# arnab39/Semi-supervised-segmentation-cycleGAN

Hardware: AMD Instinct MI355X
Metric: training images/sec (G+D step) at 256x256 (higher is better)
Workload: dtype f32; 1 GPU; VOC2012 21-class 256x256 semisupervised_cycleGAN as-written G+D step, batch=8 per GPU, fp32 tensors, 3-piece split-bf16 contraction, fp32-accurate (six exact bf16 piece products per fp32 product on the bf16 matrix cores, fp32 accumulation - forward, data and weight gradients; 21 / 20-channel stems and heads zero-padded onto the same contraction, 1- / 3-channel ends on the exact fp32 MFMA); global_batch=8, image_unit=one labeled + one unlabeled 256x256 image, parallelism=dp1, losses_finite=True

## Files before the change

### include/sscg.h

```cpp
#ifndef SSCG_H
#define SSCG_H
#include <stddef.h>
#include <stdint.h>

#ifdef __cplusplus
extern "C" {
#endif

#define SSCG_ABI_VERSION 18

#define SSCG_F32 0
#define SSCG_BF16 1
#define SSCG_BF16X3 2

#define SSCG_ERR_BAD_ARG (-1)
#define SSCG_ERR_UNSUPPORTED (-2)
#define SSCG_ERR_WORKSPACE (-3)

#define SSCG_ACT_NONE 0
#define SSCG_ACT_RELU 1
#define SSCG_ACT_LRELU 2
#define SSCG_ACT_TANH 3

#define SSCG_PAD_ZEROS 0
#define SSCG_PAD_REFLECT 1

int sscg_abi_version(void);
int sscg_set_dry_run(int on);

typedef struct sscg_conv_desc {
    int32_t N, H, W, C;
    int32_t K, R, S;
    int32_t P, Q;
    int32_t stride, pad, dil;
    int32_t pad_mode;
    int32_t act;
    float slope;
    int32_t x_dtype;
    int32_t w_dtype;
    int32_t y_dtype;
    int32_t precision;
    int32_t tuning;
    int64_t w_plane;
    int32_t wgrad_tuning;
} sscg_conv_desc;

size_t sscg_conv2d_fwd_workspace(const sscg_conv_desc* d);
int sscg_conv2d_fwd(const sscg_conv_desc* d, const void* x, const void* w, const float* bias, void* y, void* ws,
                    size_t ws_bytes, void* stream);

size_t sscg_conv2d_fwd_stats_bytes(const sscg_conv_desc* d, int G, int64_t L);
size_t sscg_conv2d_fwd_stats_workspace(const sscg_conv_desc* d);
int sscg_conv2d_fwd_stats(const sscg_conv_desc* d, const void* x, const void* w, const float* bias, void* y, int G, int64_t L,
                          void* stats, size_t stats_bytes, void* ws, size_t ws_bytes, void* stream);
int sscg_norm_stats_from_conv(const sscg_conv_desc* d, const void* stats, int G, int64_t L, float eps, float* mean, float* rstd,
                              float* running_mean, float* running_var, float momentum, void* stream);

int sscg_conv2d_fwd_affine_applies(const sscg_conv_desc* d);
int sscg_conv2d_fwd_affine(const sscg_conv_desc* d, const void* x, const void* w, const float* bias, const float* running_mean,
                           const float* running_var, float eps, const float* gamma, const float* beta, const void* residual, void* y,
                           void* ws, size_t ws_bytes, void* stream);

int sscg_conv2d_front_applies(const sscg_conv_desc* d, int cin);
int sscg_conv2d_front_fwd(const sscg_conv_desc* d, const void* xf, int cin, const float* w1, const float* b1, float slope1, void* h1,
                          const void* w, const float* bias, void* y, int G, int64_t L, void* stats, size_t stats_bytes, void* stream);

size_t sscg_conv2d_dgrad_workspace(const sscg_conv_desc* d);
int sscg_conv2d_dgrad(const sscg_conv_desc* d, const void* dy, const void* wt, const float* bias, void* dx,
                      int act, float slope, void* ws, size_t ws_bytes, void* stream);

size_t sscg_conv2d_wgrad_workspace(const sscg_conv_desc* d);
int sscg_conv2d_wgrad(const sscg_conv_desc* d, const void* x, const void* dy, float* dw, float beta, void* ws,
                      size_t ws_bytes, void* stream);

int sscg_weight_krsc_to_crsk(const void* w, int w_dtype, void* wt, int wt_dtype, int K, int RS, int C, void* stream);
typedef struct sscg_wt_job {
    const void* w;
    void* wt;
    int32_t w_dtype, wt_dtype;
    int32_t K, RS, C;
    int32_t block0;
} sscg_wt_job;
int sscg_weight_krsc_to_crsk_batch(const sscg_wt_job* jobs, int n_jobs, int n_blocks, void* stream);
int sscg_split3(const float* src, void* dst, int64_t n, int64_t plane_stride, void* stream);
int sscg_conv2d_split_applies(const sscg_conv_desc* d, int kind);
int sscg_cast(const void* src, int src_dtype, void* dst, int dst_dtype, int64_t n, void* stream);

size_t sscg_colsum_workspace(int64_t rows, int cols);
int sscg_colsum(const void* x, int dtype, float* out, int64_t rows, int cols, float beta, void* ws, size_t ws_bytes, void* stream);

size_t sscg_norm_stats_workspace(int G, int64_t L, int C);
int sscg_norm_stats(const void* x, int dtype, int G, int64_t L, int C, float eps, float* mean, float* rstd,
                    float* running_mean, float* running_var, float momentum, void* ws, size_t ws_bytes, void* stream);
int sscg_norm_apply(const void* x, const float* mean, const float* rstd, const float* gamma, const float* beta,
                    const void* residual, void* y, int dtype, int G, int64_t L, int C, int act, float slope, void* stream);
size_t sscg_conv2d_dgrad_bsums_bytes(const sscg_conv_desc* d, int G, int64_t L);
int sscg_conv2d_dgrad_bsums(const sscg_conv_desc* d, const void* dy, const void* wt, void* dx, const void* nx, const void* nz,
                            const void* addend, const float* mean, const float* rstd, const float* gamma, const float* beta, int G,
                            int64_t L, int act, float slope, void* sums, size_t sums_bytes, void* ws, size_t ws_bytes, void* stream);
int sscg_conv2d_dgrad_add_applies(const sscg_conv_desc* d);
int sscg_conv2d_dgrad_add(const sscg_conv_desc* d, const void* dy, const void* wt, const void* addend, void* dx, void* ws,
                          size_t ws_bytes, void* stream);
int sscg_norm_bwd_from_sums(const sscg_conv_desc* d, const void* sums, const void* dy, const void* x, const void* y, const float* mean,
                            const float* rstd, const float* gamma, const float* beta, void* dx, void* dres, float* dgamma, float* dbeta,
                            int dtype, int G, int64_t L, int C, int act, float slope, int flags, void* ws, size_t ws_bytes, void* stream);

int sscg_rstd_from_var(const float* var, float* rstd, int n, float eps, void* stream);
size_t sscg_norm_bwd_workspace(int G, int64_t L, int C);
int sscg_norm_bwd(const void* dy, const void* x, const void* y, const float* mean, const float* rstd,
                  const float* gamma, const float* beta, void* dx, void* dres, float* dgamma, float* dbeta, int dtype, int G,
                  int64_t L, int C, int act, float slope, int stats_grad, void* ws, size_t ws_bytes, void* stream);

int sscg_norm_head_applies(int C);
int sscg_norm_head_fwd(const void* x, int dtype, const float* mean, const float* rstd, const float* gamma, const float* beta,
                       const float* w, const float* bias, float* out, int G, int64_t L, int C, int act, float slope, void* stream);
size_t sscg_norm_head_bwd_workspace(int G, int64_t L, int C);
int sscg_norm_head_bwd(const float* dout, const float* w, const void* x, const float* mean, const float* rstd, const float* gamma,
                       const float* beta, void* dx, float* dw, float* dbias, float* dgamma, float* dbeta, int dtype, int G, int64_t L,
                       int C, int act, float slope, int flags, void* ws, size_t ws_bytes, void* stream);

int sscg_act_fwd(const void* x, void* y, int dtype, int64_t n, int act, float slope, void* stream);
int sscg_act_bwd(const void* dy, const void* y, void* dx, int dtype, int64_t n, int act, float slope, void* stream);
int sscg_add(const void* a, const void* b, void* y, int dtype, int64_t n, void* stream);
int sscg_resize_channels(const float* src, float* dst, int64_t rows, int Cs, int Cd, void* stream);
int sscg_dropout(const void* x, void* y, int dtype, int64_t n, float p, uint64_t seed, void* stream);
int sscg_gauss_noise(const float* x, float* y, int64_t n, float sigma, uint64_t seed, void* stream);
int sscg_maxpool2x2_fwd(const void* x, void* y, uint8_t* idx, int dtype, int N, int H, int W, int C, void* stream);
int sscg_maxpool2x2_bwd(const void* dy, const uint8_t* idx, void* dx, int dtype, int N, int H, int W, int C, void* stream);
int sscg_maxpool3x3s2_fwd(const void* x, void* y, uint8_t* idx, int dtype, int N, int H, int W, int C, int P, int Q, void* stream);
int sscg_maxpool3x3s2_bwd(const void* dy, const uint8_t* idx, void* dx, int dtype, int N, int H, int W, int C, int P, int Q, void* stream);
int sscg_upsample_bilinear_fwd(const float* x, float* y, int N, int H, int W, int C, int OH, int OW, void* stream);
int sscg_upsample_bilinear_bwd(const float* dy, float* dx, int N, int H, int W, int C, int OH, int OW, void* stream);
int sscg_reflect_pad(const void* x, void* y, int dtype, int N, int H, int W, int C, int pad, void* stream);
int sscg_reflect_pad_bwd(const void* dy, void* dx, int dtype, int N, int H, int W, int C, int pad, void* stream);
int sscg_nchw_to_nhwc(const float* x, float* y, int N, int C, int H, int W, void* stream);
int sscg_nhwc_to_nchw(const float* x, float* y, int N, int C, int H, int W, void* stream);

int sscg_softmax_fwd(const float* x, float* y, int64_t rows, int C, void* stream);
int sscg_softmax_bwd(const float* dy, const float* y, float* dx, int64_t rows, int C, void* stream);
int sscg_argmax_onehot(const float* x, float* onehot, int64_t* index, int64_t rows, int C, void* stream);
int sscg_label_onehot(const int64_t* labels, float* onehot, int64_t rows, int C, void* stream);
int sscg_confusion_hist(const int64_t* label_true, const int64_t* label_pred, int64_t n, int C, int64_t* hist, void* stream);

int sscg_image_u8_to_f32(const uint8_t* src, float* dst, int64_t rows, int C, const float* mean, const float* stdev, void* stream);
int sscg_label_lut(const uint8_t* src, int64_t* dst, int64_t n, const int64_t* lut256, void* stream);

size_t sscg_loss_workspace(int64_t n);
int sscg_ce_fwd(const float* logits, const int64_t* labels, int64_t rows, int C, float* loss, float* valid, void* ws,
                size_t ws_bytes, void* stream);
int sscg_ce_bwd(const float* logits, const int64_t* labels, int64_t rows, int C, const float* gscale, float w,
                const float* valid, float* dx, void* stream);
size_t sscg_upsample_head_workspace(int N, int H, int W);
int sscg_upsample_head_fwd(const float* x, const int64_t* labels, float* y_soft, float* loss, float* valid, float* dlogits, int N, int H,
                           int W, int C, int OH, int OW, void* ws, size_t ws_bytes, void* stream);
int sscg_upsample_head_bwd(const float* x, const float* dy_soft, const float* dlogits, const float* g_ce, const float* valid, float* dx,
                           int N, int H, int W, int C, int OH, int OW, void* stream);
int sscg_predict_head(const float* x, int N, int H, int W, int C, int OH, int OW, int64_t* index, uint8_t* label_u8,
                      const int64_t* label_true, int64_t* hist, void* stream);
int sscg_image_head(const float* x, int N, int H, int W, int C, int OH, int OW, float* y_nhwc, uint8_t* rgb_u8, void* stream);
int sscg_mse_const_fwd(const float* x, int64_t n, float target, float* loss, void* ws, size_t ws_bytes, void* stream);
int sscg_mse_const_bwd(const float* x, int64_t n, float target, const float* gscale, float w, float* dx, void* stream);
int sscg_mse_fwd(const float* a, const float* b, int64_t n, float* loss, void* ws, size_t ws_bytes, void* stream);
int sscg_mse_bwd(const float* a, const float* b, int64_t n, const float* gscale, float w, float* da, float* db, void* stream);
int sscg_l1_fwd(const float* a, const float* b, int64_t n, float* loss, void* ws, size_t ws_bytes, void* stream);
int sscg_l1_bwd(const float* a, const float* b, int64_t n, const float* gscale, float w, float* da, void* stream);
int sscg_weighted_sum(const float* const* terms, const float* w, int n, float* out, void* stream);

int sscg_adam_step(float* param, const float* grad, float* exp_avg, float* exp_avg_sq, void* shadow, int shadow_dtype, int64_t n,
                   double lr, double beta1, double beta2, double eps, int step, float grad_scale, void* stream);
int sscg_fill(float* x, int64_t n, float v, void* stream);

#ifdef __cplusplus
}
#endif
#endif
```

### semi-supervised-segmentation-cyclegan_amd/_lib.py

```python
import ctypes as C
import os

_HERE = os.path.dirname(os.path.abspath(__file__))
LIB_PATH = os.environ.get("SSCG_LIB") or os.path.join(_HERE, "libsscg.so")

ABI_VERSION = 18

F32, BF16, BF16X3 = 0, 1, 2

ACT_NONE, ACT_RELU, ACT_LRELU, ACT_TANH = 0, 1, 2, 3
PAD_ZEROS, PAD_REFLECT = 0, 1


class ConvDesc(C.Structure):

    _fields_ = [
        ("N", C.c_int32), ("H", C.c_int32), ("W", C.c_int32), ("C", C.c_int32),
        ("K", C.c_int32), ("R", C.c_int32), ("S", C.c_int32),
        ("P", C.c_int32), ("Q", C.c_int32),
        ("stride", C.c_int32), ("pad", C.c_int32), ("dil", C.c_int32),
        ("pad_mode", C.c_int32), ("act", C.c_int32), ("slope", C.c_float),
        ("x_dtype", C.c_int32), ("w_dtype", C.c_int32), ("y_dtype", C.c_int32), ("precision", C.c_int32),
        ("tuning", C.c_int32), ("w_plane", C.c_int64), ("wgrad_tuning", C.c_int32),
    ]


_p = C.c_void_p
_i = C.c_int
_i64 = C.c_int64
_f = C.c_float
_sz = C.c_size_t
_dp = C.POINTER(ConvDesc)

SIGNATURES = {
    "sscg_abi_version": (_i, []),
    "sscg_set_dry_run": (_i, [_i]),
    "sscg_resize_channels": (_i, [_p, _p, _i64, _i, _i, _p]),
    "sscg_conv2d_fwd_workspace": (_sz, [_dp]),
    "sscg_conv2d_fwd": (_i, [_dp, _p, _p, _p, _p, _p, _sz, _p]),
    "sscg_conv2d_fwd_stats_bytes": (_sz, [_dp, _i, _i64]),
    "sscg_conv2d_fwd_stats_workspace": (_sz, [_dp]),
    "sscg_conv2d_fwd_stats": (_i, [_dp, _p, _p, _p, _p, _i, _i64, _p, _sz, _p, _sz, _p]),
    "sscg_norm_stats_from_conv": (_i, [_dp, _p, _i, _i64, _f, _p, _p, _p, _p, _f, _p]),
    "sscg_conv2d_fwd_affine_applies": (_i, [_dp]),
    "sscg_conv2d_fwd_affine": (_i, [_dp, _p, _p, _p, _p, _p, _f, _p, _p, _p, _p, _p, _sz, _p]),
    "sscg_conv2d_front_applies": (_i, [_dp, _i]),
    "sscg_conv2d_front_fwd": (_i, [_dp, _p, _i, _p, _p, _f, _p, _p, _p, _p, _i, _i64, _p, _sz, _p]),
    "sscg_conv2d_dgrad_workspace": (_sz, [_dp]),
    "sscg_conv2d_dgrad": (_i, [_dp, _p, _p, _p, _p, _i, _f, _p, _sz, _p]),
    "sscg_conv2d_dgrad_bsums_bytes": (_sz, [_dp, _i, _i64]),
    "sscg_conv2d_dgrad_bsums": (_i, [_dp, _p, _p, _p, _p, _p, _p, _p, _p, _p, _p, _i, _i64, _i, _f, _p, _sz, _p, _sz, _p]),
    "sscg_conv2d_dgrad_add_applies": (_i, [_dp]),
    "sscg_conv2d_dgrad_add": (_i, [_dp, _p, _p, _p, _p, _p, _sz, _p]),
    "sscg_norm_bwd_from_sums": (_i, [_dp, _p, _p, _p, _p, _p, _p, _p, _p, _p, _p, _p, _p, _i, _i, _i64, _i, _i, _f, _i, _p, _sz, _p]),
    "sscg_conv2d_wgrad_workspace": (_sz, [_dp]),
    "sscg_conv2d_wgrad": (_i, [_dp, _p, _p, _p, _f, _p, _sz, _p]),
    "sscg_weight_krsc_to_crsk": (_i, [_p, _i, _p, _i, _i, _i, _i, _p]),
    "sscg_weight_krsc_to_crsk_batch": (_i, [_p, _i, _i, _p]),
    "sscg_split3": (_i, [_p, _p, _i64, _i64, _p]),
    "sscg_conv2d_split_applies": (_i, [_dp, _i]),
    "sscg_cast": (_i, [_p, _i, _p, _i, _i64, _p]),
    "sscg_colsum_workspace": (_sz, [_i64, _i]),
    "sscg_colsum": (_i, [_p, _i, _p, _i64, _i, _f, _p, _sz, _p]),
    "sscg_norm_stats_workspace": (_sz, [_i, _i64, _i]),
    "sscg_norm_stats": (_i, [_p, _i, _i, _i64, _i, _f, _p, _p, _p, _p, _f, _p, _sz, _p]),
    "sscg_norm_apply": (_i, [_p, _p, _p, _p, _p, _p, _p, _i, _i, _i64, _i, _i, _f, _p]),
    "sscg_rstd_from_var": (_i, [_p, _p, _i, _f, _p]),
    "sscg_norm_bwd_workspace": (_sz, [_i, _i64, _i]),
    "sscg_norm_bwd": (_i, [_p, _p, _p, _p, _p, _p, _p, _p, _p, _p, _p, _i, _i, _i64, _i, _i, _f, _i, _p, _sz, _p]),
    "sscg_norm_head_applies": (_i, [_i]),
    "sscg_norm_head_fwd": (_i, [_p, _i, _p, _p, _p, _p, _p, _p, _p, _i, _i64, _i, _i, _f, _p]),
    "sscg_norm_head_bwd_workspace": (_sz, [_i, _i64, _i]),
    "sscg_norm_head_bwd": (_i, [_p, _p, _p, _p, _p, _p, _p, _p, _p, _p, _p, _p, _i, _i, _i64, _i, _i, _f, _i, _p, _sz, _p]),
    "sscg_act_fwd": (_i, [_p, _p, _i, _i64, _i, _f, _p]),
    "sscg_act_bwd": (_i, [_p, _p, _p, _i, _i64, _i, _f, _p]),
    "sscg_add": (_i, [_p, _p, _p, _i, _i64, _p]),
    "sscg_dropout": (_i, [_p, _p, _i, _i64, _f, C.c_uint64, _p]),
    "sscg_gauss_noise": (_i, [_p, _p, _i64, _f, C.c_uint64, _p]),
    "sscg_maxpool2x2_fwd": (_i, [_p, _p, _p, _i, _i, _i, _i, _i, _p]),
    "sscg_maxpool2x2_bwd": (_i, [_p, _p, _p, _i, _i, _i, _i, _i, _p]),
    "sscg_maxpool3x3s2_fwd": (_i, [_p, _p, _p, _i, _i, _i, _i, _i, _i, _i, _p]),
    "sscg_maxpool3x3s2_bwd": (_i, [_p, _p, _p, _i, _i, _i, _i, _i, _i, _i, _p]),
    "sscg_upsample_bilinear_fwd": (_i, [_p, _p, _i, _i, _i, _i, _i, _i, _p]),
    "sscg_upsample_bilinear_bwd": (_i, [_p, _p, _i, _i, _i, _i, _i, _i, _p]),
    "sscg_reflect_pad": (_i, [_p, _p, _i, _i, _i, _i, _i, _i, _p]),
    "sscg_reflect_pad_bwd": (_i, [_p, _p, _i, _i, _i, _i, _i, _i, _p]),
    "sscg_nchw_to_nhwc": (_i, [_p, _p, _i, _i, _i, _i, _p]),
    "sscg_nhwc_to_nchw": (_i, [_p, _p, _i, _i, _i, _i, _p]),
    "sscg_softmax_fwd": (_i, [_p, _p, _i64, _i, _p]),
    "sscg_softmax_bwd": (_i, [_p, _p, _p, _i64, _i, _p]),
    "sscg_argmax_onehot": (_i, [_p, _p, _p, _i64, _i, _p]),
    "sscg_label_onehot": (_i, [_p, _p, _i64, _i, _p]),
    "sscg_confusion_hist": (_i, [_p, _p, _i64, _i, _p, _p]),
    "sscg_image_u8_to_f32": (_i, [_p, _p, _i64, _i, _p, _p, _p]),
    "sscg_label_lut": (_i, [_p, _p, _i64, _p, _p]),
    "sscg_loss_workspace": (_sz, [_i64]),
    "sscg_ce_fwd": (_i, [_p, _p, _i64, _i, _p, _p, _p, _sz, _p]),
    "sscg_ce_bwd": (_i, [_p, _p, _i64, _i, _p, _f, _p, _p, _p]),
    "sscg_upsample_head_workspace": (_sz, [_i, _i, _i]),
    "sscg_upsample_head_fwd": (_i, [_p, _p, _p, _p, _p, _p, _i, _i, _i, _i, _i, _i, _p, _sz, _p]),
    "sscg_upsample_head_bwd": (_i, [_p, _p, _p, _p, _p, _p, _i, _i, _i, _i, _i, _i, _p]),
    "sscg_predict_head": (_i, [_p, _i, _i, _i, _i, _i, _i, _p, _p, _p, _p, _p]),
    "sscg_image_head": (_i, [_p, _i, _i, _i, _i, _i, _i, _p, _p, _p]),
    "sscg_mse_const_fwd": (_i, [_p, _i64, _f, _p, _p, _sz, _p]),
    "sscg_mse_const_bwd": (_i, [_p, _i64, _f, _p, _f, _p, _p]),
    "sscg_mse_fwd": (_i, [_p, _p, _i64, _p, _p, _sz, _p]),
    "sscg_mse_bwd": (_i, [_p, _p, _i64, _p, _f, _p, _p, _p]),
    "sscg_l1_fwd": (_i, [_p, _p, _i64, _p, _p, _sz, _p]),
    "sscg_l1_bwd": (_i, [_p, _p, _i64, _p, _f, _p, _p]),
    "sscg_weighted_sum": (_i, [C.POINTER(_p), C.POINTER(_f), _i, _p, _p]),
    "sscg_adam_step": (_i, [_p, _p, _p, _p, _p, _i, _i64, C.c_double, C.c_double, C.c_double, C.c_double, _i, _f, _p]),
    "sscg_fill": (_i, [_p, _i64, _f, _p]),
}


class SscgError(RuntimeError):
    pass


def _load():
    if not os.path.exists(LIB_PATH):
        raise ImportError(
            "libsscg.so not found at %s - build it with `make -C %s/csrc` or "
            "`python -c 'import __graft_entry__ as g; g.build()'`. There is no fallback path." % (LIB_PATH, _HERE))
    lib = C.CDLL(LIB_PATH)
    for name, (res, args) in SIGNATURES.items():
        fn = getattr(lib, name)
        fn.restype = res
        fn.argtypes = args
    v = lib.sscg_abi_version()
    if v != ABI_VERSION:
        raise ImportError("libsscg.so ABI version %d != binding version %d" % (v, ABI_VERSION))
    if os.environ.get("SSCG_TRACE"):
        return _Traced(lib)
    if os.environ.get("SSCG_RACECHECK"):
        racecheck = dev_tool("racecheck")
        racecheck.install()
        return racecheck._Checked(lib)
    if os.environ.get("SSCG_FUZZ"):
        return dev_tool("racecheck")._Fuzzed(lib)
    return lib


def dev_tool(name):
    import importlib.util
    import sys
    if name in sys.modules:
        return sys.modules[name]
    path = os.path.join(os.path.dirname(_HERE), "tools", name + ".py")
    spec = importlib.util.spec_from_file_location(name, path)
    if spec is None or not os.path.exists(path):
        raise ImportError("development tool %s not found at %s" % (name, path))
    mod = importlib.util.module_from_spec(spec)
    sys.modules[name] = mod
    spec.loader.exec_module(mod)
    return mod


class _Traced:

    def __init__(self, lib):
        self._lib = lib

    def __getattr__(self, name):
        fn = getattr(self._lib, name)

        def call(*a):
            import sys
            import torch
            sys.stderr.write("[sscg] %s%s\n" % (name, tuple(x if isinstance(x, (int, float)) else "." for x in a)))
            sys.stderr.flush()
            r = fn(*a)
            if torch.cuda.is_available():
                torch.cuda.synchronize()
            return r
        return call


lib = _load()

_ERRS = {-1: "SSCG_ERR_BAD_ARG", -2: "SSCG_ERR_UNSUPPORTED", -3: "SSCG_ERR_WORKSPACE"}


def check(rc, what):
    if rc != 0:
        raise SscgError("%s failed: %s" % (what, _ERRS.get(rc, "hipError_t %d" % rc)))
```

### semi-supervised-segmentation-cyclegan_amd/csrc/common.h

```cpp
#pragma once
#include <hip/hip_runtime.h>
#include <stdint.h>
#include <stddef.h>

extern int g_sscg_dry_run;
#undef hipLaunchKernelGGL
#define hipLaunchKernelGGL(kernelName, numBlocks, numThreads, memPerBlock, streamId, ...)                                   \
    do {                                                                                                                     \
        if (!g_sscg_dry_run) { (kernelName)<<<(numBlocks), (numThreads), (memPerBlock), (streamId)>>>(__VA_ARGS__); }        \
    } while (0)

typedef float f32x16 __attribute__((ext_vector_type(16)));
typedef __bf16 bf16x8 __attribute__((ext_vector_type(8)));

struct sscg_bf3 { __bf16 h, m, l; };
__device__ __forceinline__ sscg_bf3 sscg_split3(float x) {
    sscg_bf3 t;
    t.h = (__bf16)x;
    const float r1 = x - (float)t.h;
    t.m = (__bf16)r1;
    const float r2 = r1 - (float)t.m;
    t.l = (__bf16)r2;
    return t;
}
typedef float f32x4 __attribute__((ext_vector_type(4)));
typedef __bf16 bf16x4 __attribute__((ext_vector_type(4)));

typedef uint32_t sscg_u32x4 __attribute__((ext_vector_type(4)));
__device__ __forceinline__ uint32_t sscg_cvt_pk_bf16(float a, float b) {
    typedef __bf16 bf16x2_t __attribute__((ext_vector_type(2)));
    typedef float f32x2_t __attribute__((ext_vector_type(2)));
    const f32x2_t v = {a, b};
    return __builtin_bit_cast(uint32_t, __builtin_convertvector(v, bf16x2_t));
}
__device__ __forceinline__ void sscg_split8(const float (&x)[8], bf16x8& h, bf16x8& m, bf16x8& l) {
    sscg_u32x4 ph, pm, pl;
#pragma unroll
    for (int w = 0; w < 4; ++w) {
        const float a = x[2 * w], b = x[2 * w + 1];
        const uint32_t hh = sscg_cvt_pk_bf16(a, b);
        const float ra = a - __builtin_bit_cast(float, hh << 16), rb = b - __builtin_bit_cast(float, hh & 0xffff0000u);
        const uint32_t mm = sscg_cvt_pk_bf16(ra, rb);
        const float sa = ra - __builtin_bit_cast(float, mm << 16), sb = rb - __builtin_bit_cast(float, mm & 0xffff0000u);
        ph[w] = hh; pm[w] = mm; pl[w] = sscg_cvt_pk_bf16(sa, sb);
    }
    h = __builtin_bit_cast(bf16x8, ph);
    m = __builtin_bit_cast(bf16x8, pm);
    l = __builtin_bit_cast(bf16x8, pl);
}

template <typename T> __device__ __forceinline__ float ld1(const T* p);
template <> __device__ __forceinline__ float ld1<float>(const float* p) { return *p; }
template <> __device__ __forceinline__ float ld1<__bf16>(const __bf16* p) { return (float)*p; }
template <typename T> __device__ __forceinline__ void st1(T* p, float v);
template <> __device__ __forceinline__ void st1<float>(float* p, float v) { *p = v; }
template <> __device__ __forceinline__ void st1<__bf16>(__bf16* p, float v) { *p = (__bf16)v; }
template <typename T> __device__ __forceinline__ void ld4(const T* p, float v[4]);
template <> __device__ __forceinline__ void ld4<float>(const float* p, float v[4]) {
    const f32x4 t = *reinterpret_cast<const f32x4*>(p);
    v[0] = t[0]; v[1] = t[1]; v[2] = t[2]; v[3] = t[3];
}
template <> __device__ __forceinline__ void ld4<__bf16>(const __bf16* p, float v[4]) {
    const bf16x4 t = *reinterpret_cast<const bf16x4*>(p);
    v[0] = (float)t[0]; v[1] = (float)t[1]; v[2] = (float)t[2]; v[3] = (float)t[3];
}
template <typename T> __device__ __forceinline__ void st4(T* p, const float v[4]);
template <> __device__ __forceinline__ void st4<float>(float* p, const float v[4]) {
    const f32x4 t = {v[0], v[1], v[2], v[3]};
    *reinterpret_cast<f32x4*>(p) = t;
}
template <> __device__ __forceinline__ void st4<__bf16>(__bf16* p, const float v[4]) {
    const bf16x4 t = {(__bf16)v[0], (__bf16)v[1], (__bf16)v[2], (__bf16)v[3]};
    *reinterpret_cast<bf16x4*>(p) = t;
}
typedef __bf16 bf16x8_t __attribute__((ext_vector_type(8)));
template <typename T> __device__ __forceinline__ void ld8(const T* p, float v[8]);
template <> __device__ __forceinline__ void ld8<float>(const float* p, float v[8]) { ld4<float>(p, v); ld4<float>(p + 4, v + 4); }
template <> __device__ __forceinline__ void ld8<__bf16>(const __bf16* p, float v[8]) {
    const bf16x8_t t = *reinterpret_cast<const bf16x8_t*>(p);
#pragma unroll
    for (int e = 0; e < 8; ++e) v[e] = (float)t[e];
}
template <typename T> __device__ __forceinline__ void st8(T* p, const float v[8]);
template <> __device__ __forceinline__ void st8<float>(float* p, const float v[8]) { st4<float>(p, v); st4<float>(p + 4, v + 4); }
template <> __device__ __forceinline__ void st8<__bf16>(__bf16* p, const float v[8]) {
    bf16x8_t t;
#pragma unroll
    for (int e = 0; e < 8; ++e) t[e] = (__bf16)v[e];
    *reinterpret_cast<bf16x8_t*>(p) = t;
}

#define SSCG_OK 0
#define SSCG_ERR_BAD_ARG (-1)
#define SSCG_ERR_UNSUPPORTED (-2)
#define SSCG_ERR_WORKSPACE (-3)

#define SSCG_LAUNCH_CHECK()                        \
    do {                                           \
        hipError_t e__ = hipGetLastError();        \
        if (e__ != hipSuccess) return (int)e__;    \
    } while (0)

enum { SSCG_ACT_NONE = 0, SSCG_ACT_RELU = 1, SSCG_ACT_LRELU = 2, SSCG_ACT_TANH = 3 };

__device__ __forceinline__ float sscg_act(float v, int act, float slope) {
    if (act == SSCG_ACT_RELU) return v > 0.f ? v : 0.f;
    if (act == SSCG_ACT_LRELU) return v > 0.f ? v : v * slope;
    if (act == SSCG_ACT_TANH) return tanhf(v);
    return v;
}

struct FastDiv {
    uint32_t mul;
    uint32_t shift;
    int32_t d;
};

static inline FastDiv make_fastdiv(int d) {
    FastDiv f;
    f.d = d;
    uint32_t l = 0;
    while ((1u << l) < (uint32_t)d) ++l;
    f.shift = l;
    f.mul = (uint32_t)((((uint64_t)1 << 32) * (((uint64_t)1 << l) - (uint64_t)d)) / (uint64_t)d + 1);
    return f;
}

__device__ __forceinline__ int fd_div(int n, const FastDiv& f) {
    return (int)((__umulhi((uint32_t)n, f.mul) + (uint32_t)n) >> f.shift);
}

__device__ __forceinline__ int xcd_remap(int bid, int nwg) {
    const int q = nwg >> 3, r = nwg & 7;
    const int xcd = bid & 7, idx = bid >> 3;
    return (xcd < r ? xcd * (q + 1) : r * (q + 1) + (xcd - r) * q) + idx;
}

static inline int cdiv(long a, long b) { return (int)((a + b - 1) / b); }

__device__ __forceinline__ double wave_sum(double v) {
#pragma unroll
    for (int o = 32; o > 0; o >>= 1) v += __shfl_xor(v, o, 64);
    return v;
}
__device__ __forceinline__ float wave_sum(float v) {
#pragma unroll
    for (int o = 32; o > 0; o >>= 1) v += __shfl_xor(v, o, 64);
    return v;
}

#define SSCG_ENSURE_SMEM(kern, smem)                                                                                                   \
    do {                                                                                                                               \
        static size_t sscg_attr_smem_[16] = {0};                                                                                       \
        int sscg_dev_ = 0;                                                                                                             \
        if (hipGetDevice(&sscg_dev_) != hipSuccess) sscg_dev_ = 0;                                                                     \
        size_t& sscg_cur_ = sscg_attr_smem_[sscg_dev_ & 15];                                                                           \
        if (sscg_cur_ == 0) sscg_cur_ = 64 * 1024;                                                                                     \
        if ((size_t)(smem) > sscg_cur_) {                                                                                              \
            hipError_t sscg_e_ = hipFuncSetAttribute(reinterpret_cast<const void*>(kern), hipFuncAttributeMaxDynamicSharedMemorySize, \
                                                     (int)(smem));                                                                     \
            if (sscg_e_ != hipSuccess) return (int)sscg_e_;                                                                            \
            sscg_cur_ = (size_t)(smem);                                                                                                \
        }                                                                                                                              \
    } while (0)

template <int BM, int BN, int NT, int TM, int TN>
__device__ __forceinline__ void sscg_stage_store_tile(const f32x16 (&acc)[TM][TN], float* ot, float* __restrict__ out, int m0, int n0, int Mlim,
                                                      int Ng, int row_w, int col_w, int li, int lh, int tid, float beta) {
    constexpr int OLD = BN + 4;
    __syncthreads();
#pragma unroll
    for (int j = 0; j < TN; ++j)
#pragma unroll
        for (int i = 0; i < TM; ++i)
#pragma unroll
            for (int e = 0; e < 16; ++e)
                ot[(row_w + i * 32 + (e & 3) + 8 * (e >> 2) + 4 * lh) * OLD + col_w + j * 32 + li] = acc[i][j][e];
    __syncthreads();
    constexpr int TPR = BN / 4;
    constexpr int RPP = NT / TPR;
    const int c4 = (tid % TPR) * 4;
    const int n = n0 + c4;
    if (n >= Ng) return;
#pragma unroll
    for (int ps = 0; ps < BM / RPP; ++ps) {
        const int r = tid / TPR + ps * RPP;
        const int m = m0 + r;
        if (m >= Mlim) break;
        f32x4 v = *reinterpret_cast<const f32x4*>(ot + r * OLD + c4);
        float* o = out + (size_t)m * Ng + n;
        if (beta != 0.f) v += beta * *reinterpret_cast<const f32x4*>(o);
        *reinterpret_cast<f32x4*>(o) = v;
    }
}
```

### semi-supervised-segmentation-cyclegan_amd/csrc/conv_split.hip

```cpp
#include "common.h"
#include "sscg_internal.h"
#include "reduce_common.h"
#include "bn_fold.h"
#include <cstdlib>
#include <type_traits>

namespace {

#ifndef KS_ABLATE
#define KS_ABLATE 0
#endif
#ifndef KS_BUFLD
#define KS_BUFLD 1
#endif
#ifndef KS_ACC2
#define KS_ACC2 1
#endif
#ifndef KS_LATE_WAIT
#define KS_LATE_WAIT 0
#endif
#ifndef KS_LB4
#define KS_LB4 1
#endif
constexpr int BKS = 32;
// ... 1754 lines not shown
#pragma unroll
            for (int pl = 0; pl < 3; ++pl) {
                asm volatile("ds_read_b64_tr_b16 %0, %1 offset:%2" : "=v"(fb[j][pl][0]) : "v"(lds0 + b_off[j]), "n"(pl * WS_PLANE));
                asm volatile("ds_read_b64_tr_b16 %0, %1 offset:%2" : "=v"(fb[j][pl][1]) : "v"(lds0 + b_off[j]), "n"(pl * WS_PLANE + 4 * WS_ROWB));
            }
        if (next) read_raw((it + 1) % WF_NRAW);
        __builtin_amdgcn_sched_barrier(0);
        wait_lgkm<0>();
        bf16x8 va[TM][3], vb[TN][3];
#pragma unroll
        for (int i = 0; i < TM; ++i)
#pragma unroll
            for (int pl = 0; pl < 3; ++pl) {
                va[i][pl] = __builtin_shufflevector(fa[i][pl][0], fa[i][pl][1], 0, 1, 2, 3, 4, 5, 6, 7);
                pin(va[i][pl]);
            }
#pragma unroll
        for (int j = 0; j < TN; ++j)
#pragma unroll
            for (int pl = 0; pl < 3; ++pl) {
                vb[j][pl] = __builtin_shufflevector(fb[j][pl][0], fb[j][pl][1], 0, 1, 2, 3, 4, 5, 6, 7);
                pin(vb[j][pl]);
            }
        if (next) { pin(raw[0][0]); pin(raw[0][1]); pin(raw[1][0]); pin(raw[1][1]); }
        __builtin_amdgcn_sched_barrier(0);
#pragma unroll
        for (int t = 0; t < 6; ++t) {
            const int ap = t == 0 ? 2 : (t == 1 || t == 3) ? 1 : 0;
            const int bp = (t == 0 || t == 3 || t == 5) ? 0 : (t == 1 || t == 4) ? 1 : 2;
#pragma unroll
            for (int i = 0; i < TM; ++i)
#pragma unroll
                for (int j = 0; j < TN; ++j)
                    acc[i][j] = __builtin_amdgcn_mfma_f32_32x32x16_bf16(va[i][ap], vb[j][bp], acc[i][j], 0, 0, 0);
            if (t == 0) {
                __builtin_amdgcn_sched_barrier(0);
                if (next) split_raw();
            }
        }
        if (next) {
#pragma unroll
            for (int n = 0; n < 20; ++n) {
                __builtin_amdgcn_sched_group_barrier(0x008, 1, 0);
                __builtin_amdgcn_sched_group_barrier(0x002, 5, 0);
            }
#pragma unroll
            for (int op = 0; op < 2; ++op)
#pragma unroll
                for (int pl = 0; pl < 3; ++pl) pin(pc[op][pl]);
        }
        __builtin_amdgcn_sched_barrier(0);
        if (!next) break;
        __builtin_amdgcn_s_barrier();
        if (issued < nsteps) { request_tile(); ++issued; }
        write_pieces();
        wait_lgkm<0>();
        if (it + 2 < nsteps) wait_tile(it + 2);
        __builtin_amdgcn_s_barrier();
    }

    float* out = p.out + (size_t)split * p.Kc * p.C;
    const bool direct = (p.splits == 1);
    ws_store_tile(acc, reinterpret_cast<float*>(smem_raw), out, m0, n0, p.Kc, p.C, row_w, col_w, li, lh, tid, direct ? p.beta : 0.f);
}

struct WgsPlan { int splits, chunk; };

WgsPlan plan_wgs(const sscg_conv_desc* d) {
    const int Kc = d->K, Ng = d->R * d->S * d->C;
    const long npix = (long)d->N * d->P * d->Q;
    const long steps = cdiv(npix, WS_BKP);
    const long tiles = (long)cdiv(Kc, 128) * cdiv(Ng, 128);
    const int force = (d->wgrad_tuning >> 8) & 0xffff;
    const bool two_stages = ((d->wgrad_tuning >> 24) & 1) != 0;
    long s = force > 0 ? force : (two_stages ? 768 : 512) / tiles;
    if (s > steps / 8) s = steps / 8;
    if (s > 1024) s = 1024;
    if (s < 1) s = 1;
    WgsPlan pl;
    pl.chunk = (int)(cdiv(steps, s) * WS_BKP);
    pl.splits = cdiv(npix, pl.chunk);
    return pl;
}

WgsPlan plan_wgf(const sscg_conv_desc* d) {
    const long npix = (long)d->N * d->P * d->Q;
    const long steps = cdiv(npix, WS_BKP);
    const long tiles = (long)cdiv(d->K, 128) * cdiv(d->C, 128);
    const int force = (d->wgrad_tuning >> 8) & 0xffff;
    long s = force > 0 ? force : 512 / tiles;
    if (s > steps / 8) s = steps / 8;
    if (s > 1024) s = 1024;
    if (s < 1) s = 1;
    WgsPlan pl;
    pl.chunk = (int)(cdiv(steps, s) * WS_BKP);
    pl.splits = cdiv(npix, pl.chunk);
    return pl;
}

bool wgf_applies(const sscg_conv_desc* d) {
    const int cls = d->wgrad_tuning & 0xff;
    if (cls == 3 || cls == 4 || cls == 5) return false;
    if ((long)d->K * d->C >= (1L << 21)) return false;
    const long npix = (long)d->N * d->P * d->Q;
    if (npix * (d->K > d->C ? d->K : d->C) * 4 >= (1L << 31)) return false;
    return d->R == 1 && d->S == 1 && d->stride == 1 && d->pad == 0 && d->K >= 128 && d->C >= 128 && d->K % 8 == 0 && d->C % 8 == 0 &&
           npix >= 1024;
}

int launch_wgf(const sscg_conv_desc* d, const void* x, const void* dy, float* dw, float beta, void* ws, size_t ws_bytes, hipStream_t st) {
    const WgsPlan pl = plan_wgf(d);
    const size_t part = pl.splits > 1 ? (size_t)pl.splits * d->K * d->C * sizeof(float) : 0;
    if (part && (!ws || ws_bytes < part)) return SSCG_ERR_WORKSPACE;
    WgfParams p = {};
    p.x = reinterpret_cast<const float*>(x); p.dy = reinterpret_cast<const float*>(dy);
    p.out = pl.splits > 1 ? reinterpret_cast<float*>(ws) : dw;
    p.Kc = d->K; p.C = d->C;
    p.npix = d->N * d->P * d->Q; p.chunk = pl.chunk;
    p.tiles_n = cdiv(p.C, 128); p.tiles = cdiv(p.Kc, 128) * p.tiles_n; p.splits = pl.splits;
    p.beta = pl.splits > 1 ? 0.f : beta;
    SSCG_ENSURE_SMEM(wgradf_kernel, WF_SMEM);
    hipLaunchKernelGGL(wgradf_kernel, dim3(p.tiles * pl.splits), dim3(256), WF_SMEM, st, p);
    SSCG_LAUNCH_CHECK();
    if (pl.splits > 1) return sscg_wgrad_reduce(reinterpret_cast<const float*>(ws), dw, (size_t)d->K * d->C, pl.splits, beta, st);
    return SSCG_OK;
}

}

static size_t wgs_planes_bytes(const sscg_conv_desc* d) {
    return ((size_t)d->N * d->H * d->W * d->C + (size_t)d->N * d->P * d->Q * d->K) * 3 * sizeof(bf16);
}

bool sscg_wgrads_applies(const sscg_conv_desc* d) {
    if (d->precision != 2 || d->x_dtype != SSCG_F32 || d->y_dtype != SSCG_F32) return false;
    if (wgf_applies(d)) return true;
    if ((d->wgrad_tuning & 0xff) == 3) return false;
    const int Ng = d->R * d->S * d->C;
    if ((d->wgrad_tuning & 0xff) != 4 && d->R * d->S == 1 && (long)d->K * d->C < (1L << 21)) return false;
    if (wgs_planes_bytes(d) > ((size_t)3 << 29)) return false;
    return d->K >= 128 && Ng >= 128 && d->K % 8 == 0 && d->C % 8 == 0 && (long)d->N * d->P * d->Q >= 1024;
}

size_t sscg_wgrads_workspace(const sscg_conv_desc* d) {
    if (wgf_applies(d)) {
        const WgsPlan pf = plan_wgf(d);
        return pf.splits > 1 ? (size_t)pf.splits * d->K * d->C * sizeof(float) : 0;
    }
    const WgsPlan pl = plan_wgs(d);
    const size_t part = pl.splits > 1 ? (size_t)pl.splits * d->K * d->R * d->S * d->C * sizeof(float) : 0;
    return ((wgs_planes_bytes(d) + 255) & ~(size_t)255) + part;
}

int sscg_wgrads(const sscg_conv_desc* d, const void* x, const void* dy, float* dw, float beta, void* ws, size_t ws_bytes, hipStream_t st) {
    if (wgf_applies(d)) return launch_wgf(d, x, dy, dw, beta, ws, ws_bytes, st);
    if (!ws || ws_bytes < sscg_wgrads_workspace(d)) return SSCG_ERR_WORKSPACE;
    const WgsPlan pl = plan_wgs(d);
    const size_t nx = (size_t)d->N * d->H * d->W * d->C, ny = (size_t)d->N * d->P * d->Q * d->K;
    bf16* x3 = reinterpret_cast<bf16*>(ws);
    bf16* y3 = x3 + 3 * nx;
    float* part = reinterpret_cast<float*>(reinterpret_cast<char*>(ws) + ((wgs_planes_bytes(d) + 255) & ~(size_t)255));
    hipLaunchKernelGGL(split3_kernel, dim3(cdiv((long)((nx + 7) / 8), 256)), dim3(256), 0, st, reinterpret_cast<const float*>(x), x3, nx, nx);
    hipLaunchKernelGGL(split3_kernel, dim3(cdiv((long)((ny + 7) / 8), 256)), dim3(256), 0, st, reinterpret_cast<const float*>(dy), y3, ny, ny);
    SSCG_LAUNCH_CHECK();
    WgsParams p = {};
    p.x3 = x3; p.dy3 = y3; p.xplane = (long)nx; p.yplane = (long)ny;
    p.out = pl.splits > 1 ? part : dw;
    p.Kc = d->K; p.Ng = d->R * d->S * d->C; p.C = d->C;
    p.H = d->H; p.W = d->W; p.P = d->P; p.Q = d->Q; p.S = d->S;
    p.stride = d->stride; p.pad = d->pad; p.dil = d->dil; p.pad_mode = d->pad_mode;
    p.npix = d->N * d->P * d->Q; p.chunk = pl.chunk;
    p.tiles_n = cdiv(p.Ng, 128); p.tiles = cdiv(p.Kc, 128) * p.tiles_n; p.splits = pl.splits;
    p.beta = pl.splits > 1 ? 0.f : beta;
    p.div_pq = make_fastdiv(d->P * d->Q);
    p.div_q = make_fastdiv(d->Q);
    if ((d->wgrad_tuning >> 24) & 1) {
        const size_t smem2 = (size_t)128 * 132 * sizeof(float);
        SSCG_ENSURE_SMEM(wgrads_kernel<2>, smem2);
        hipLaunchKernelGGL(wgrads_kernel<2>, dim3(p.tiles * pl.splits), dim3(256), smem2, st, p);
    } else {
        const size_t smem = (size_t)3 * WS_STAGE;
        SSCG_ENSURE_SMEM(wgrads_kernel<3>, smem);
        hipLaunchKernelGGL(wgrads_kernel<3>, dim3(p.tiles * pl.splits), dim3(256), smem, st, p);
    }
    SSCG_LAUNCH_CHECK();
    if (pl.splits > 1) return sscg_wgrad_reduce(part, dw, (size_t)d->K * p.Ng, pl.splits, beta, st);
    return SSCG_OK;
}
```

### semi-supervised-segmentation-cyclegan_amd/csrc/conv_wgrad.hip

```cpp
#include "common.h"
#include <cstdlib>
#include "sscg_internal.h"

namespace {

constexpr int BKP = 32;

struct WgParams {
    const void* __restrict__ x;
    const void* __restrict__ dy;
    float* __restrict__ out;
    int Kc;
    int Ng;
    int C;
    int H, W, P, Q;
    int S;
    int stride, pad, dil, pad_mode;
    int npix;
    int chunk;
    int tiles_n;
    int tiles;
    int splits;
    float beta;
    FastDiv div_pq, div_q;
// ... 459 lines not shown
    const int q = threadIdx.x % wq;
    const int pl = threadIdx.x / wq;
    float acc[T][4];
#pragma unroll
    for (int t = 0; t < T; ++t)
#pragma unroll
        for (int e = 0; e < 4; ++e) acc[t][e] = 0.f;
    if (pl < lanes) {
        const int stride = lanes * gridDim.x;
        int px = blockIdx.x * lanes + pl;
        for (; px + stride < p.npix; px += 2 * stride) {
            float w0[4], w1[4];
            ld4<TW>(wide + (size_t)px * p.Wd + q * 4, w0);
            ld4<TW>(wide + (size_t)(px + stride) * p.Wd + q * 4, w1);
            const TT* th0 = thin + (size_t)px * T;
            const TT* th1 = thin + (size_t)(px + stride) * T;
#pragma unroll
            for (int t = 0; t < T; ++t) {
                const float v0 = ld1<TT>(th0 + t), v1 = ld1<TT>(th1 + t);
#pragma unroll
                for (int e = 0; e < 4; ++e) acc[t][e] = fmaf(v1, w1[e], fmaf(v0, w0[e], acc[t][e]));
            }
        }
        if (px < p.npix) {
            float w0[4];
            ld4<TW>(wide + (size_t)px * p.Wd + q * 4, w0);
            const TT* th0 = thin + (size_t)px * T;
#pragma unroll
            for (int t = 0; t < T; ++t) {
                const float v0 = ld1<TT>(th0 + t);
#pragma unroll
                for (int e = 0; e < 4; ++e) acc[t][e] = fmaf(v0, w0[e], acc[t][e]);
            }
        }
    }
#pragma unroll
    for (int t0 = 0; t0 < T; t0 += TB) {
        if (pl < lanes) {
#pragma unroll
            for (int t = 0; t < TB; ++t)
                if (t0 + t < T)
#pragma unroll
                    for (int e = 0; e < 4; ++e) red[((size_t)pl * TB + t) * p.Wd + q * 4 + e] = acc[t0 + t][e];
        }
        __syncthreads();
        const int nt = (T - t0) < TB ? (T - t0) : TB;
        for (int i = threadIdx.x; i < nt * p.Wd; i += 256) {
            float s = 0.f;
            for (int l = 0; l < lanes; ++l) s += red[(size_t)l * TB * p.Wd + i];
            p.part[(size_t)blockIdx.x * T * p.Wd + (size_t)t0 * p.Wd + i] = s;
        }
        __syncthreads();
    }
}

__global__ __launch_bounds__(256) void thin_wgrad_reduce_kernel(const float* __restrict__ part, float* __restrict__ dw, int blocks,
                                                                 int T, int Wd, int K, int C, float beta) {
    const int o = blockIdx.x * 4 + (threadIdx.x >> 6);
    const int lane = threadIdx.x & 63;
    if (o >= T * Wd) return;
    float s = 0.f;
    for (int b = lane; b < blocks; b += 64) s += part[(size_t)b * T * Wd + o];
    s = wave_sum(s);
    if (lane == 0) {
        const int t = o / Wd, w = o - t * Wd;
        const int k = (K == T && K <= C) ? t : w;
        const int c = (K == T && K <= C) ? w : t;
        float* d = dw + (size_t)k * C + c;
        *d = beta != 0.f ? beta * *d + s : s;
    }
}

bool thin_wgrad_applies(const sscg_conv_desc* d) {
    if (d->R != 1 || d->S != 1 || d->stride != 1 || d->pad != 0 || d->pad_mode != 0) return false;
    const int T = d->K < d->C ? d->K : d->C, Wd = d->K < d->C ? d->C : d->K;
    return T <= THIN_MAX && Wd % 4 == 0 && Wd <= 256 && Wd >= 16 && (long)d->N * d->H * d->W >= 65536;
}

template <int T, typename TW, typename TT>
int launch_thin(const ThinParams& p, int blocks, size_t smem, hipStream_t st) {
    SSCG_ENSURE_SMEM((thin_wgrad_kernel<T, TW, TT>), smem);
    hipLaunchKernelGGL((thin_wgrad_kernel<T, TW, TT>), dim3(blocks), dim3(256), smem, st, p);
    return SSCG_OK;
}

template <typename TW, typename TT>
int launch_thin_T(const ThinParams& p, size_t smem, hipStream_t st) {
    switch (p.T) {
        case 1: return launch_thin<1, TW, TT>(p, THIN_BLOCKS, smem, st);
        case 2: return launch_thin<2, TW, TT>(p, THIN_BLOCKS, smem, st);
        case 3: return launch_thin<3, TW, TT>(p, THIN_BLOCKS, smem, st);
        case 4: return launch_thin<4, TW, TT>(p, THIN_BLOCKS, smem, st);
        case 20: return launch_thin<20, TW, TT>(p, THIN_BLOCKS, smem, st);
        case 21: return launch_thin<21, TW, TT>(p, THIN_BLOCKS, smem, st);
        default: return SSCG_ERR_UNSUPPORTED;
    }
}

int thin_wgrad(const sscg_conv_desc* d, const void* x, const void* dy, float* dw, float beta, void* ws, hipStream_t st) {
    const bool thin_is_k = d->K <= d->C;
    ThinParams p;
    p.T = thin_is_k ? d->K : d->C;
    p.Wd = thin_is_k ? d->C : d->K;
    p.wide = thin_is_k ? x : dy;
    p.thin = thin_is_k ? dy : x;
    const int wide_dt = thin_is_k ? d->x_dtype : d->y_dtype, thin_dt = thin_is_k ? d->y_dtype : d->x_dtype;
    p.part = reinterpret_cast<float*>(ws);
    p.npix = d->N * d->H * d->W;
    const int lanes = 256 / (p.Wd / 4);
    const size_t smem = (size_t)lanes * (p.T < 4 ? p.T : 4) * p.Wd * sizeof(float);
    int rc;
    if (wide_dt == SSCG_F32 && thin_dt == SSCG_F32) rc = launch_thin_T<float, float>(p, smem, st);
    else if (wide_dt == SSCG_BF16 && thin_dt == SSCG_F32) rc = launch_thin_T<__bf16, float>(p, smem, st);
    else if (wide_dt == SSCG_BF16 && thin_dt == SSCG_BF16) rc = launch_thin_T<__bf16, __bf16>(p, smem, st);
    else rc = SSCG_ERR_UNSUPPORTED;
    if (rc) return rc;
    SSCG_LAUNCH_CHECK();
    hipLaunchKernelGGL(thin_wgrad_reduce_kernel, dim3(cdiv(p.T * p.Wd, 4)), dim3(256), 0, st, p.part, dw, THIN_BLOCKS, p.T, p.Wd,
                       d->K, d->C, beta);
    SSCG_LAUNCH_CHECK();
    return SSCG_OK;
}

bool thin_wgrad_supported_T(int T) { return T == 1 || T == 2 || T == 3 || T == 4 || T == 20 || T == 21; }

}

int sscg_wgrad_reduce(const float* ws, float* dw, size_t n, int splits, float beta, hipStream_t st) {
    static const bool w4 = !(getenv("SSCG_WGRAD_REDUCE_W4") && atoi(getenv("SSCG_WGRAD_REDUCE_W4")) == 0);
    const bool vec_ok = n % 4 == 0 && ((size_t)dw & 15) == 0 && ((size_t)ws & 15) == 0;
    if (vec_ok && w4 && splits >= 8 && n / 4 <= 64 * 16384)
        hipLaunchKernelGGL(wgrad_reduce_w4_kernel, dim3(cdiv((long)(n / 4), 64)), dim3(256), 0, st, ws, dw, n, splits, beta);
    else if (vec_ok)
        hipLaunchKernelGGL(wgrad_reduce_kernel<4>, dim3(cdiv((long)(n / 4), 256)), dim3(256), 0, st, ws, dw, n, splits, beta);
    else
        hipLaunchKernelGGL(wgrad_reduce_kernel<1>, dim3(cdiv((long)n, 256)), dim3(256), 0, st, ws, dw, n, splits, beta);
    SSCG_LAUNCH_CHECK();
    return SSCG_OK;
}

static bool wg_dt_ok(int dt) { return dt == SSCG_F32 || dt == SSCG_BF16; }

extern "C" size_t sscg_conv2d_wgrad_workspace(const sscg_conv_desc* d) {
    if (!d) return 0;
    if (thin_wgrad_applies(d) && thin_wgrad_supported_T(d->K < d->C ? d->K : d->C))
        return (size_t)THIN_BLOCKS * d->K * d->C * sizeof(float);
    if (sscg_wgrad16_applies(d)) return sscg_wgrad16_workspace(d);
    if (sscg_wgrads_applies(d)) return sscg_wgrads_workspace(d);
    WgPlan pl = plan_wgrad(d);
    if (pl.splits <= 1) return 0;
    return (size_t)pl.splits * d->K * d->R * d->S * d->C * sizeof(float);
}

extern "C" int sscg_conv2d_wgrad(const sscg_conv_desc* d, const void* x, const void* dy, float* dw, float beta,
                                 void* ws, size_t ws_bytes, void* stream) {
    if (!d || !x || !dy || !dw) return SSCG_ERR_BAD_ARG;
    if (d->N <= 0 || d->C <= 0 || d->K <= 0 || !wg_dt_ok(d->x_dtype) || !wg_dt_ok(d->y_dtype)) return SSCG_ERR_BAD_ARG;
    if ((long)d->N * d->H * d->W * (long)d->C >= (1L << 31)) return SSCG_ERR_UNSUPPORTED;
    if ((long)d->N * d->P * d->Q * (long)d->K >= (1L << 31)) return SSCG_ERR_UNSUPPORTED;
    hipStream_t st = (hipStream_t)stream;
    if (thin_wgrad_applies(d) && thin_wgrad_supported_T(d->K < d->C ? d->K : d->C)) {
        if (!ws || ws_bytes < sscg_conv2d_wgrad_workspace(d)) return SSCG_ERR_WORKSPACE;
        return thin_wgrad(d, x, dy, dw, beta, ws, st);
    }
    if (sscg_wgrad16_applies(d)) return sscg_wgrad16(d, x, dy, dw, beta, ws, ws_bytes, st);
    if (sscg_wgrads_applies(d)) return sscg_wgrads(d, x, dy, dw, beta, ws, ws_bytes, st);
    WgPlan pl = plan_wgrad(d);
    size_t need = pl.splits > 1 ? (size_t)pl.splits * d->K * d->R * d->S * d->C * sizeof(float) : 0;
    if (need > 0 && (!ws || ws_bytes < need)) return SSCG_ERR_WORKSPACE;
    WgParams p;
    p.x = x; p.dy = dy;
    p.out = pl.splits > 1 ? reinterpret_cast<float*>(ws) : dw;
    p.Kc = d->K; p.Ng = d->R * d->S * d->C; p.C = d->C;
    p.H = d->H; p.W = d->W; p.P = d->P; p.Q = d->Q; p.S = d->S;
    p.stride = d->stride; p.pad = d->pad; p.dil = d->dil; p.pad_mode = d->pad_mode;
    p.npix = d->N * d->P * d->Q; p.chunk = pl.chunk; p.tiles_n = 0; p.tiles = 0; p.splits = 1;
    p.beta = pl.splits > 1 ? 0.f : beta;
    p.div_pq = make_fastdiv(d->P * d->Q);
    p.div_q = make_fastdiv(d->Q);
    const bool va4 = (d->K % 4 == 0), vb4 = (d->C % 4 == 0);
    int rc;
    if (d->x_dtype == SSCG_F32 && d->y_dtype == SSCG_F32) {
        if (va4 && vb4) rc = dispatch_wg<4, 4>(p, pl, d->precision, st);
        else if (va4) rc = dispatch_wg<4, 1>(p, pl, d->precision, st);
        else if (vb4) rc = dispatch_wg<1, 4>(p, pl, d->precision, st);
        else rc = dispatch_wg<1, 1>(p, pl, d->precision, st);
    } else if (d->x_dtype == SSCG_F32) {
        rc = dispatch_wg_types<float, __bf16>(p, pl, va4, vb4, st);
    } else if (d->y_dtype == SSCG_F32) {
        rc = dispatch_wg_types<__bf16, float>(p, pl, va4, vb4, st);
    } else {
        rc = SSCG_ERR_UNSUPPORTED;
    }
    if (rc) return rc;
    if (pl.splits > 1) return sscg_wgrad_reduce(reinterpret_cast<const float*>(ws), dw, (size_t)d->K * p.Ng, pl.splits, beta, st);
    return SSCG_OK;
}
```

### semi-supervised-segmentation-cyclegan_amd/csrc/norm.hip

```cpp
#include "common.h"
#include "sscg_internal.h"
#include <cstdlib>

namespace {

enum { RM_SUM = 0, RM_STATS = 1, RM_BWD = 2, RM_BWD_HEAD = 3 };

struct RedParams {
    const void* __restrict__ x;
    const void* __restrict__ dy;
    const void* __restrict__ y;
    const float* __restrict__ mean;
    const float* __restrict__ rstd;
    const float* __restrict__ gamma;
    const float* __restrict__ beta;
    double* __restrict__ part;
    const float* __restrict__ head_w;
    const float* __restrict__ head_dout;
    double* __restrict__ head_part;
    long L;
    int C;
    int chunks;
    long rows_per_chunk;
    int act;
// ... 352 lines not shown
    const int g = blockIdx.z;
    float mu[VEC], rs[VEC], ga[VEC], be[VEC];
    const size_t s = (size_t)g * p.C + c;
    ldv<float, VEC>(p.mean + s, mu);
    ldv<float, VEC>(p.rstd + s, rs);
    if (p.gamma) {
        ldv<float, VEC>(p.gamma + c, ga);
        ldv<float, VEC>(p.beta + c, be);
    }
    const size_t base = (size_t)g * p.L * p.C + c;
    const T* px = reinterpret_cast<const T*>(p.x) + base;
    const T* pr = p.res ? reinterpret_cast<const T*>(p.res) + base : nullptr;
    T* py = reinterpret_cast<T*>(p.y) + base;
    const long r_begin = (long)blockIdx.x * rows_per_chunk;
    const long r_end = r_begin + rows_per_chunk < p.L ? r_begin + rows_per_chunk : p.L;
    for (long r = r_begin + rl; r < r_end; r += (long)rw * U) {
        float xv[U][VEC], rv[U][VEC];
#pragma unroll
        for (int u = 0; u < U; ++u) {
            const long rr = r + (long)u * rw;
            if (rr < r_end) {
                ldv<T, VEC>(px + (size_t)rr * p.C, xv[u]);
                if (pr) ldv<T, VEC>(pr + (size_t)rr * p.C, rv[u]);
            }
        }
#pragma unroll
        for (int u = 0; u < U; ++u) {
            const long rr = r + (long)u * rw;
            if (rr < r_end) {
                float out[VEC];
#pragma unroll
                for (int e = 0; e < VEC; ++e) {
                    float v = (xv[u][e] - mu[e]) * rs[e];
                    if (p.gamma) v = v * ga[e] + be[e];
                    if (pr) v += rv[u][e];
                    out[e] = sscg_act(v, p.act, p.slope);
                }
                stv<T, VEC>(py + (size_t)rr * p.C, out);
            }
        }
    }
}

struct SlabPlan { bool ok; int cw_shift, slabs, chunks, rows_per_chunk; };
static SlabPlan plan_slab(int G, long L, int C, int vec, int U) {
    SlabPlan pl = {false, 0, 1, 1, 0};
    static const bool off = getenv("SSCG_NORM_SLAB") && atoi(getenv("SSCG_NORM_SLAB")) == 0;
    if (off || vec < 4 || C % vec) return pl;
    const int cg = C / vec;
    if (cg & (cg - 1)) return pl;
    int sh = 0;
    while ((1 << sh) < cg && sh < 8) ++sh;
    pl.cw_shift = sh;
    pl.slabs = cg >> sh;
    const int rw = 256 >> sh;
    const long round = (long)rw * U;
    long chunks = (L + round - 1) / round;
    long budget = 4096 / ((long)G * pl.slabs);
    if (budget < 1) budget = 1;
    if (chunks > budget) chunks = budget;
    long rpc = (L + chunks - 1) / chunks;
    rpc = (rpc + round - 1) / round * round;
    pl.chunks = (int)((L + rpc - 1) / rpc);
    pl.rows_per_chunk = (int)rpc;
    if (G > 65535 || pl.slabs > 65535 || rpc > 0x7fffffffL) return pl;
    pl.ok = true;
    return pl;
}

struct BwdApplyParams {
    const void* __restrict__ dy;
    const void* __restrict__ x;
    const void* __restrict__ y;
    const float* __restrict__ mean;
    const float* __restrict__ rstd;
    const float* __restrict__ gamma;
    const float* __restrict__ beta;
    const float* __restrict__ coef;
    const float* __restrict__ head_w;
    const float* __restrict__ head_dout;
    void* __restrict__ dx;
    void* __restrict__ dres;
    long L;
    int C;
    int act;
    float slope;
    uint32_t total;
    FastDiv div_cg;
    FastDiv div_l;
};

template <typename T, int VEC>
__global__ __launch_bounds__(256) void norm_bwd_apply_kernel(BwdApplyParams p) {
    const int CG = p.C / VEC;
    const T* pdy = reinterpret_cast<const T*>(p.dy);
    const T* px = reinterpret_cast<const T*>(p.x);
    const T* py = reinterpret_cast<const T*>(p.y);
    T* pdx = reinterpret_cast<T*>(p.dx);
    T* pdres = reinterpret_cast<T*>(p.dres);
    for (uint32_t i = blockIdx.x * 256 + threadIdx.x; i < p.total; i += gridDim.x * 256) {
        const int row = fd_div((int)i, p.div_cg);
        const int c = ((int)i - row * CG) * VEC;
        const int g = fd_div(row, p.div_l);
        const size_t o = (size_t)i * VEC;
        const bool remask = p.act != SSCG_ACT_NONE && py == nullptr;
        float dv[VEC], xv[VEC], yv[VEC];
        if (p.head_w) {
            float hw[VEC];
            ldv<float, VEC>(p.head_w + c, hw);
            const float d = p.head_dout[row];
#pragma unroll
            for (int e = 0; e < VEC; ++e) dv[e] = d * hw[e];
        } else {
            ldv<T, VEC>(pdy + o, dv);
        }
        ldv<T, VEC>(px + o, xv);
        if (p.act != SSCG_ACT_NONE && !remask) ldv<T, VEC>(py + o, yv);
        float gx[VEC], gr[VEC];
        float mu[VEC], rsv[VEC], ga[VEC], be[VEC], c1[VEC], c2[VEC];
        const size_t s = (size_t)g * p.C + c;
        ldv<float, VEC>(p.rstd + s, rsv);
#pragma unroll
        for (int e = 0; e < VEC; ++e) { ga[e] = 1.f; be[e] = 0.f; mu[e] = 0.f; c1[e] = 0.f; c2[e] = 0.f; }
        if (p.gamma) ldv<float, VEC>(p.gamma + c, ga);
        if (remask && p.beta) ldv<float, VEC>(p.beta + c, be);
        if (p.coef || remask) ldv<float, VEC>(p.mean + s, mu);
        if (p.coef) {
            if constexpr (VEC == 1) {
                c1[0] = p.coef[s * 2]; c2[0] = p.coef[s * 2 + 1];
            } else {
                float kk[2 * VEC];
#pragma unroll
                for (int q = 0; q < 2 * VEC; q += 4) ld4<float>(p.coef + s * 2 + q, kk + q);
#pragma unroll
                for (int e = 0; e < VEC; ++e) { c1[e] = kk[2 * e]; c2[e] = kk[2 * e + 1]; }
            }
        }
#pragma unroll
        for (int e = 0; e < VEC; ++e) {
            const float xh = (xv[e] - mu[e]) * rsv[e];
            float ym = yv[e];
            if (remask) ym = xh * ga[e] + be[e];
            float gg = p.act != SSCG_ACT_NONE ? act_grad(dv[e], ym, p.act, p.slope) : dv[e];
            gr[e] = gg;
            float v = gg;
            if (p.coef) v = gg - c1[e] - xh * c2[e];
            gx[e] = v * rsv[e] * ga[e];
        }
        stv<T, VEC>(pdx + o, gx);
        if (p.dres) stv<T, VEC>(pdres + o, gr);
    }
}

template <typename T, int VEC, int U>
__global__ __launch_bounds__(256) void norm_bwd_apply_slab_kernel(BwdApplyParams p, int cw_shift, int rows_per_chunk) {
    const int tid = threadIdx.x;
    const int col = tid & ((1 << cw_shift) - 1), rl = tid >> cw_shift, rw = 256 >> cw_shift;
    const int c = (((int)blockIdx.y << cw_shift) + col) * VEC;
    const int g = blockIdx.z;
    const bool remask = p.act != SSCG_ACT_NONE && p.y == nullptr;
    const bool has_y = p.act != SSCG_ACT_NONE && !remask;
    float mu[VEC], rsv[VEC], ga[VEC], be[VEC], c1[VEC], c2[VEC], hw[VEC];
    const size_t s = (size_t)g * p.C + c;
    ldv<float, VEC>(p.rstd + s, rsv);
#pragma unroll
    for (int e = 0; e < VEC; ++e) { ga[e] = 1.f; be[e] = 0.f; mu[e] = 0.f; c1[e] = 0.f; c2[e] = 0.f; hw[e] = 0.f; }
    if (p.gamma) ldv<float, VEC>(p.gamma + c, ga);
    if (remask && p.beta) ldv<float, VEC>(p.beta + c, be);
    if (p.coef || remask) ldv<float, VEC>(p.mean + s, mu);
    if (p.coef) {
        float kk[2 * VEC];
#pragma unroll
        for (int q = 0; q < 2 * VEC; q += 4) ld4<float>(p.coef + s * 2 + q, kk + q);
#pragma unroll
        for (int e = 0; e < VEC; ++e) { c1[e] = kk[2 * e]; c2[e] = kk[2 * e + 1]; }
    }
    if (p.head_w) ldv<float, VEC>(p.head_w + c, hw);
    const size_t base = (size_t)g * p.L * p.C + c;
    const T* pdy = p.head_w ? nullptr : reinterpret_cast<const T*>(p.dy) + base;
    const T* px = reinterpret_cast<const T*>(p.x) + base;
    const T* py = has_y ? reinterpret_cast<const T*>(p.y) + base : nullptr;
    T* pdx = reinterpret_cast<T*>(p.dx) + base;
    T* pdres = p.dres ? reinterpret_cast<T*>(p.dres) + base : nullptr;
    const float* pdo = p.head_w ? p.head_dout + (size_t)g * p.L : nullptr;
    const long r_begin = (long)blockIdx.x * rows_per_chunk;
    const long r_end = r_begin + rows_per_chunk < p.L ? r_begin + rows_per_chunk : p.L;
    for (long r = r_begin + rl; r < r_end; r += (long)rw * U) {
        float dv[U][VEC], xv[U][VEC], yv[U][VEC];
#pragma unroll
        for (int u = 0; u < U; ++u) {
            const long rr = r + (long)u * rw;
            if (rr < r_end) {
                const size_t o = (size_t)rr * p.C;
                if (p.head_w) {
                    const float d = pdo[rr];
#pragma unroll
                    for (int e = 0; e < VEC; ++e) dv[u][e] = d * hw[e];
                } else {
                    ldv<T, VEC>(pdy + o, dv[u]);
                }
                ldv<T, VEC>(px + o, xv[u]);
                if (has_y) ldv<T, VEC>(py + o, yv[u]);
            }
        }
#pragma unroll
        for (int u = 0; u < U; ++u) {
            const long rr = r + (long)u * rw;
            if (rr < r_end) {
                const size_t o = (size_t)rr * p.C;
                float gx[VEC], gr[VEC];
#pragma unroll
                for (int e = 0; e < VEC; ++e) {
                    const float xh = (xv[u][e] - mu[e]) * rsv[e];
                    float ym = yv[u][e];
                    if (remask) ym = xh * ga[e] + be[e];
                    float gg = p.act != SSCG_ACT_NONE ? act_grad(dv[u][e], ym, p.act, p.slope) : dv[u][e];
                    gr[e] = gg;
                    float v = gg;
                    if (p.coef) v = gg - c1[e] - xh * c2[e];
                    gx[e] = v * rsv[e] * ga[e];
                }
                stv<T, VEC>(pdx + o, gx);
                if (pdres) stv<T, VEC>(pdres + o, gr);
            }
        }
    }
}

struct HeadParams {
    const void* __restrict__ x;
    const float* __restrict__ mean;
    const float* __restrict__ rstd;
    const float* __restrict__ gamma;
    const float* __restrict__ beta;
    const float* __restrict__ w;
    const float* __restrict__ bias;
    float* __restrict__ out;
    long L;
    long rows;
    int C;
    int act;
    float slope;
};

template <typename T>
__global__ __launch_bounds__(256) void norm_head_fwd_kernel(HeadParams p) {
    const int lanes = p.C >> 2;
    const int rows_per_wave = 64 / lanes;
    const int lane = threadIdx.x & 63;
    const int sub = lane / lanes;
    const int c = (lane - sub * lanes) * 4;
    const T* px = reinterpret_cast<const T*>(p.x);
    float w[4], ga[4] = {1.f, 1.f, 1.f, 1.f}, be[4] = {0.f, 0.f, 0.f, 0.f};
    ld4<float>(p.w + c, w);
    if (p.gamma) { ld4<float>(p.gamma + c, ga); ld4<float>(p.beta + c, be); }
    const float b0 = p.bias ? p.bias[0] : 0.f;
    const long wave = (long)blockIdx.x * 4 + (threadIdx.x >> 6);
    const long nwaves = (long)gridDim.x * 4;
    constexpr int U = 4;
    for (long r0 = wave * rows_per_wave * U; r0 < p.rows; r0 += nwaves * rows_per_wave * U) {
        float xv[U][4], mu[U][4], rs[U][4];
        long r[U];
#pragma unroll
        for (int u = 0; u < U; ++u) {
            r[u] = r0 + (long)u * rows_per_wave + sub;
            const long rr = r[u] < p.rows ? r[u] : p.rows - 1;
            const long g = rr / p.L;
            ld4<T>(px + (size_t)rr * p.C + c, xv[u]);
            ld4<float>(p.mean + (size_t)g * p.C + c, mu[u]);
            ld4<float>(p.rstd + (size_t)g * p.C + c, rs[u]);
        }
#pragma unroll
        for (int u = 0; u < U; ++u) {
            float acc = 0.f;
#pragma unroll
            for (int e = 0; e < 4; ++e) {
                float v = (xv[u][e] - mu[u][e]) * rs[u][e];
                if (p.gamma) v = v * ga[e] + be[e];
                acc += w[e] * sscg_act(v, p.act, p.slope);
            }
            for (int m = 1; m < lanes; m <<= 1) acc += __shfl_xor(acc, m, 64);
            if (c == 0 && r[u] < p.rows) p.out[r[u]] = acc + b0;
        }
    }
}

__global__ void rstd_from_var_kernel(const float* __restrict__ var, float* __restrict__ rstd, int n, float eps) {
    int i = blockIdx.x * blockDim.x + threadIdx.x;
    if (i < n) rstd[i] = (float)(1.0 / sqrt((double)var[i] + (double)eps));
}

inline int ew_grid(size_t total) {
    size_t b = (total + 255) / 256;
    if (b > 4096) b = 4096;
    if (b < 1) b = 1;
    return (int)b;
}


struct ConvStatParams {
    const double* __restrict__ rec;
    const double* __restrict__ xrecs;
    float* __restrict__ mean;
    float* __restrict__ rstd;
    float* __restrict__ rmean;
    float* __restrict__ rvar;
    int valid_tiles;
    int BMT, RPT;
    int xrec, xgroup;
    int G, C;
    long L;
    float eps, momentum;
};

template <int CPB>
__global__ __launch_bounds__(1024) void finalize_conv_stats_kernel(ConvStatParams p) {
    constexpr int FCS_LANES = 1024 / CPB;
    __shared__ double sm[FCS_LANES][CPB][2];
    const int cl = threadIdx.x % CPB;
    const int w = threadIdx.x / CPB;
    const int c = blockIdx.x * CPB + cl;
    const bool cok = c < p.C;
    const int g0 = p.rmean ? 0 : blockIdx.y;
    const int g1 = p.rmean ? p.G : blockIdx.y + 1;
    for (int g = g0; g < g1; ++g) {
        const long lo = (long)g * p.L, hi = lo + p.L;
        const int t_first = (int)((lo + p.BMT - 1) / p.BMT);
        int t_last = (int)((hi + p.BMT - 1) / p.BMT) - 1;
        if (t_last > p.valid_tiles - 1) t_last = p.valid_tiles - 1;
        double s = 0.0, q = 0.0;
        if (cok) {
            const int n0 = (t_last - t_first + 1) * p.RPT;
            const double* base = p.rec + (((size_t)t_first * p.RPT * 2 + 0) * p.C + c) * 2;
            const size_t rstride = (size_t)2 * p.C * 2;
            int k = w;
            for (; k + 3 * FCS_LANES < n0; k += 4 * FCS_LANES) {
                const double2 e0 = *reinterpret_cast<const double2*>(base + (size_t)k * rstride);
                const double2 e1 = *reinterpret_cast<const double2*>(base + (size_t)(k + FCS_LANES) * rstride);
                const double2 e2 = *reinterpret_cast<const double2*>(base + (size_t)(k + 2 * FCS_LANES) * rstride);
                const double2 e3 = *reinterpret_cast<const double2*>(base + (size_t)(k + 3 * FCS_LANES) * rstride);
                s += (e0.x + e1.x) + (e2.x + e3.x);
                q += (e0.y + e1.y) + (e2.y + e3.y);
            }
            for (; k < n0; k += FCS_LANES) {
                const double2 e = *reinterpret_cast<const double2*>(base + (size_t)k * rstride);
                s += e.x; q += e.y;
            }
            if (g > 0 && t_first >= 1 && t_first - 1 < p.valid_tiles) {
                for (int k1 = w; k1 < p.RPT; k1 += FCS_LANES) {
                    const size_t r = (size_t)(t_first - 1) * p.RPT + k1;
                    const double2 e = *reinterpret_cast<const double2*>(p.rec + ((r * 2 + 1) * p.C + c) * 2);
                    s += e.x; q += e.y;
                }
            }
            if (p.xrec > 0 && p.xgroup == g) {
                for (int k2 = w; k2 < p.xrec; k2 += FCS_LANES) {
                    const double2 e = *reinterpret_cast<const double2*>(p.xrecs + ((size_t)k2 * p.C + c) * 2);
                    s += e.x; q += e.y;
                }
            }
        }
        sm[w][cl][0] = s; sm[w][cl][1] = q;
        __syncthreads();
#pragma unroll
        for (int st = FCS_LANES / 2; st >= 1; st >>= 1) {
            if (w < st) { sm[w][cl][0] += sm[w + st][cl][0]; sm[w][cl][1] += sm[w + st][cl][1]; }
            __syncthreads();
        }
        if (w == 0 && cok) {
            const double a = sm[0][cl][0], b = sm[0][cl][1];
            const int i = g * p.C + c;
            const double m = a / (double)p.L;
            double var = b / (double)p.L - m * m;
            if (var < 0.0) var = 0.0;
            p.mean[i] = (float)m;
            p.rstd[i] = (float)(1.0 / sqrt(var + (double)p.eps));
            if (p.rmean) {
                const double unb = p.L > 1 ? var * (double)p.L / (double)(p.L - 1) : var;
                p.rmean[c] = (float)((1.0 - (double)p.momentum) * (double)p.rmean[c] + (double)p.momentum * m);
                p.rvar[c] = (float)((1.0 - (double)p.momentum) * (double)p.rvar[c] + (double)p.momentum * unb);
            }
        }
        __syncthreads();
    }
}

}

extern "C" size_t sscg_colsum_workspace(int64_t rows, int cols) { return part_bytes(1, rows, cols); }

extern "C" int sscg_colsum(const void* x, int dtype, float* out, int64_t rows, int cols, float beta, void* ws, size_t ws_bytes,
                           void* stream) {
    if (!x || !out || rows <= 0 || cols <= 0 || (dtype != SSCG_F32 && dtype != SSCG_BF16)) return SSCG_ERR_BAD_ARG;
    if (!ws || ws_bytes < part_bytes(1, rows, cols)) return SSCG_ERR_WORKSPACE;
    hipStream_t st = (hipStream_t)stream;
    RedParams p = {};
    p.x = x; p.part = reinterpret_cast<double*>(ws); p.L = rows; p.C = cols;
    int rc = launch_reduce<RM_SUM>(p, 1, dtype, st);
    if (rc) return rc;
    RedPlan pl = plan_reduce(1, rows, cols, dtype);
    hipLaunchKernelGGL(finalize_sum_kernel, dim3(cdiv(cols, FIN_CH)), dim3(256), 0, st, p.part, out, cols, pl.chunks, beta);
    SSCG_LAUNCH_CHECK();
    return SSCG_OK;
}

extern "C" size_t sscg_norm_stats_workspace(int G, int64_t L, int C) { return part_bytes(G, L, C); }

extern "C" int sscg_norm_stats(const void* x, int dtype, int G, int64_t L, int C, float eps, float* mean, float* rstd,
                               float* running_mean, float* running_var, float momentum, void* ws, size_t ws_bytes,
                               void* stream) {
    if (!x || !mean || !rstd || G <= 0 || L <= 0 || C <= 0 || (dtype != SSCG_F32 && dtype != SSCG_BF16)) return SSCG_ERR_BAD_ARG;
    if ((running_mean != nullptr) != (running_var != nullptr)) return SSCG_ERR_BAD_ARG;
    if (!ws || ws_bytes < part_bytes(G, L, C)) return SSCG_ERR_WORKSPACE;
    hipStream_t st = (hipStream_t)stream;
    RedParams p = {};
    p.x = x; p.part = reinterpret_cast<double*>(ws); p.L = L; p.C = C;
    int rc = launch_reduce<RM_STATS>(p, G, dtype, st);
    if (rc) return rc;
    RedPlan pl = plan_reduce(G, L, C, dtype);
    hipLaunchKernelGGL(finalize_stats_kernel, dim3(cdiv(C, FIN_CH), running_mean ? 1 : G), dim3(256), 0, st, p.part, mean, rstd,
                       running_mean, running_var, G, C, pl.chunks, (long)L, eps, momentum);
    SSCG_LAUNCH_CHECK();
    return SSCG_OK;
}

int sscg_finalize_conv_stats(const double* stats, int valid_tiles, int rows_per_tile, int records_per_tile, const double* xrecs,
                             int xrec, int xgroup, int G, long L, int C, float eps, float* mean, float* rstd, float* running_mean,
                             float* running_var, float momentum, hipStream_t st) {
    ConvStatParams p = {};
    p.rec = stats; p.xrecs = xrecs; p.mean = mean; p.rstd = rstd; p.rmean = running_mean; p.rvar = running_var;
    p.valid_tiles = valid_tiles; p.BMT = rows_per_tile; p.RPT = records_per_tile; p.xrec = xrec; p.xgroup = xgroup;
    p.G = G; p.C = C; p.L = L; p.eps = eps; p.momentum = momentum;
    const int gy = running_mean ? 1 : G;
    const long recs = (L / rows_per_tile + 1) * records_per_tile;
#ifndef FCS_NARROW
#define FCS_NARROW 1
#endif
    if (FCS_NARROW && cdiv(C, 16) * gy < 64 && recs >= 512)
        hipLaunchKernelGGL(finalize_conv_stats_kernel<4>, dim3(cdiv(C, 4), gy), dim3(1024), 0, st, p);
    else
        hipLaunchKernelGGL(finalize_conv_stats_kernel<16>, dim3(cdiv(C, 16), gy), dim3(1024), 0, st, p);
    SSCG_LAUNCH_CHECK();
    return SSCG_OK;
}

template <typename T>
static void launch_apply(const ApplyParams& p, int vec, hipStream_t st, int G = 0) {
    static const int u8 = getenv("SSCG_NORM_SLAB_U8A") ? atoi(getenv("SSCG_NORM_SLAB_U8A")) : 2;
    const int U = vec == 8 ? u8 : 4;
    const SlabPlan sp = (G > 0 && U > 0) ? plan_slab(G, p.L, p.C, vec, U) : SlabPlan{false, 0, 1, 1, 0};
    if (sp.ok) {
        const dim3 grid(sp.chunks, sp.slabs, G);
        if (vec == 8 && U == 2) hipLaunchKernelGGL((norm_apply_slab_kernel<T, 8, 2>), grid, dim3(256), 0, st, p, sp.cw_shift, sp.rows_per_chunk);
        else if (vec == 8) hipLaunchKernelGGL((norm_apply_slab_kernel<T, 8, 4>), grid, dim3(256), 0, st, p, sp.cw_shift, sp.rows_per_chunk);
        else hipLaunchKernelGGL((norm_apply_slab_kernel<T, 4, 4>), grid, dim3(256), 0, st, p, sp.cw_shift, sp.rows_per_chunk);
        return;
    }
    if (vec == 8) hipLaunchKernelGGL((norm_apply_kernel<T, 8>), dim3(ew_grid(p.total)), dim3(256), 0, st, p);
    else if (vec == 4) hipLaunchKernelGGL((norm_apply_kernel<T, 4>), dim3(ew_grid(p.total)), dim3(256), 0, st, p);
    else hipLaunchKernelGGL((norm_apply_kernel<T, 1>), dim3(ew_grid(p.total)), dim3(256), 0, st, p);
}

extern "C" int sscg_norm_apply(const void* x, const float* mean, const float* rstd, const float* gamma,
                               const float* beta, const void* residual, void* y, int dtype, int G, int64_t L, int C, int act,
                               float slope, void* stream) {
    if (!x || !mean || !rstd || !y || G <= 0 || L <= 0 || C <= 0 || (dtype != SSCG_F32 && dtype != SSCG_BF16)) return SSCG_ERR_BAD_ARG;
    if ((gamma != nullptr) != (beta != nullptr)) return SSCG_ERR_BAD_ARG;
    ApplyParams p = {};
    p.x = x; p.mean = mean; p.rstd = rstd; p.gamma = gamma; p.beta = beta; p.res = residual; p.y = y;
    p.L = L; p.C = C; p.act = act; p.slope = slope;
    const int vec = vec_for(C, dtype);
    if ((size_t)G * L * C / vec >= ((size_t)1 << 31)) return SSCG_ERR_UNSUPPORTED;
    p.total = (uint32_t)((size_t)G * L * C / vec);
    p.div_cg = make_fastdiv(C / vec);
    p.div_l = make_fastdiv((int)L);
    hipStream_t st = (hipStream_t)stream;
    if (dtype == SSCG_BF16) launch_apply<__bf16>(p, vec, st, G);
    else launch_apply<float>(p, vec, st, G);
    SSCG_LAUNCH_CHECK();
    return SSCG_OK;
}

extern "C" int sscg_rstd_from_var(const float* var, float* rstd, int n, float eps, void* stream) {
    if (!var || !rstd || n <= 0) return SSCG_ERR_BAD_ARG;
    hipLaunchKernelGGL(rstd_from_var_kernel, dim3(cdiv(n, 256)), dim3(256), 0, (hipStream_t)stream, var, rstd, n, eps);
    SSCG_LAUNCH_CHECK();
    return SSCG_OK;
}

extern "C" size_t sscg_norm_bwd_workspace(int G, int64_t L, int C) {
    return part_bytes(G, L, C) + (size_t)G * C * 2 * sizeof(float);
}

template <typename T>
static void launch_bwd_apply(const BwdApplyParams& q, int vec, hipStream_t st, int G = 0) {
    static const int u8 = getenv("SSCG_NORM_SLAB_U8B") ? atoi(getenv("SSCG_NORM_SLAB_U8B")) : 1;
    const int U = vec == 8 ? u8 : 4;
    const SlabPlan sp = (G > 0 && U > 0) ? plan_slab(G, q.L, q.C, vec, U) : SlabPlan{false, 0, 1, 1, 0};
    if (sp.ok) {
        const dim3 grid(sp.chunks, sp.slabs, G);
        if (vec == 8 && U == 1) hipLaunchKernelGGL((norm_bwd_apply_slab_kernel<T, 8, 1>), grid, dim3(256), 0, st, q, sp.cw_shift, sp.rows_per_chunk);
        else if (vec == 8 && U == 2) hipLaunchKernelGGL((norm_bwd_apply_slab_kernel<T, 8, 2>), grid, dim3(256), 0, st, q, sp.cw_shift, sp.rows_per_chunk);
        else if (vec == 8) return launch_bwd_apply<T>(q, vec, st);
        else hipLaunchKernelGGL((norm_bwd_apply_slab_kernel<T, 4, 4>), grid, dim3(256), 0, st, q, sp.cw_shift, sp.rows_per_chunk);
        return;
    }
    if (vec == 8) hipLaunchKernelGGL((norm_bwd_apply_kernel<T, 8>), dim3(ew_grid(q.total)), dim3(256), 0, st, q);
    else if (vec == 4) hipLaunchKernelGGL((norm_bwd_apply_kernel<T, 4>), dim3(ew_grid(q.total)), dim3(256), 0, st, q);
    else hipLaunchKernelGGL((norm_bwd_apply_kernel<T, 1>), dim3(ew_grid(q.total)), dim3(256), 0, st, q);
}

extern "C" int sscg_norm_bwd(const void* dy, const void* x, const void* y, const float* mean, const float* rstd,
                             const float* gamma, const float* beta, void* dx, void* dres, float* dgamma, float* dbeta, int dtype, int G,
                             int64_t L, int C, int act, float slope, int stats_grad, void* ws, size_t ws_bytes, void* stream) {
    if (!dy || !x || !mean || !rstd || !dx || G <= 0 || L <= 0 || C <= 0 || (dtype != SSCG_F32 && dtype != SSCG_BF16)) return SSCG_ERR_BAD_ARG;
    if (act == SSCG_ACT_TANH && !y) return SSCG_ERR_BAD_ARG;
    if (act != SSCG_ACT_NONE && !y && dres) return SSCG_ERR_BAD_ARG;
    hipStream_t st = (hipStream_t)stream;
    const int overwrite = (stats_grad >> 1) & 1;
    stats_grad &= 1;
    const bool need_red = stats_grad || dgamma || dbeta;
    float* coef = nullptr;
    if (need_red) {
        if (!ws || ws_bytes < sscg_norm_bwd_workspace(G, L, C)) return SSCG_ERR_WORKSPACE;
        RedParams p = {};
        p.x = x; p.dy = dy; p.y = y; p.mean = mean; p.rstd = rstd; p.gamma = gamma; p.beta = beta;
        p.part = reinterpret_cast<double*>(ws); p.L = L; p.C = C; p.act = act; p.slope = slope;
        int rc = launch_reduce<RM_BWD>(p, G, dtype, st);
        if (rc) return rc;
        RedPlan pl = plan_reduce(G, L, C, dtype);
        coef = reinterpret_cast<float*>(reinterpret_cast<char*>(ws) + part_bytes(G, L, C));
        hipLaunchKernelGGL(finalize_bwd_kernel, dim3(cdiv(C, FIN_CH)), dim3(256), 0, st, p.part, coef, dgamma, dbeta, G, C,
                           pl.chunks, (long)L, overwrite);
        SSCG_LAUNCH_CHECK();
    }
    BwdApplyParams q = {};
    q.dy = dy; q.x = x; q.y = y; q.mean = mean; q.rstd = rstd; q.gamma = gamma; q.beta = beta;
    q.coef = stats_grad ? coef : nullptr;
    q.dx = dx; q.dres = dres; q.L = L; q.C = C; q.act = act; q.slope = slope;
    const int vec = vec_for(C, dtype);
    if ((size_t)G * L * C / vec >= ((size_t)1 << 31)) return SSCG_ERR_UNSUPPORTED;
    q.total = (uint32_t)((size_t)G * L * C / vec);
    q.div_cg = make_fastdiv(C / vec);
    q.div_l = make_fastdiv((int)L);
    if (dtype == SSCG_BF16) launch_bwd_apply<__bf16>(q, vec, st, G);
    else launch_bwd_apply<float>(q, vec, st, G);
    SSCG_LAUNCH_CHECK();
    return SSCG_OK;
}

extern "C" int sscg_norm_bwd_from_sums(const sscg_conv_desc* d, const void* sums, const void* dy, const void* x, const void* y,
                                       const float* mean, const float* rstd, const float* gamma, const float* beta, void* dx, void* dres,
                                       float* dgamma, float* dbeta, int dtype, int G, int64_t L, int C, int act, float slope, int flags,
                                       void* ws, size_t ws_bytes, void* stream) {
    if (!d || !sums || !dy || !x || !mean || !rstd || !dx || G <= 0 || L <= 0 || C <= 0 || (dtype != SSCG_F32 && dtype != SSCG_BF16)) return SSCG_ERR_BAD_ARG;
    if (act != SSCG_ACT_NONE && act != SSCG_ACT_RELU && act != SSCG_ACT_LRELU) return SSCG_ERR_UNSUPPORTED;
    if (act != SSCG_ACT_NONE && !y && dres) return SSCG_ERR_BAD_ARG;
    int bm, wm, chunks;
    if (!sscg_bsums_records(d, G, L, &bm, &wm, &chunks) || d->C != C) return SSCG_ERR_UNSUPPORTED;
    if (!ws || ws_bytes < (size_t)G * C * 2 * sizeof(float)) return SSCG_ERR_WORKSPACE;
    hipStream_t st = (hipStream_t)stream;
    float* coef = reinterpret_cast<float*>(ws);
    hipLaunchKernelGGL(finalize_bwd_kernel, dim3(cdiv(C, FIN_CH)), dim3(256), 0, st, reinterpret_cast<const double*>(sums), coef, dgamma,
                       dbeta, G, C, chunks, (long)L, (flags >> 1) & 1, bm, wm);
    SSCG_LAUNCH_CHECK();
    BwdApplyParams q = {};
    q.dy = dy; q.x = x; q.y = y; q.mean = mean; q.rstd = rstd; q.gamma = gamma; q.beta = beta;
    q.coef = coef;
    q.dx = dx; q.dres = dres; q.L = L; q.C = C; q.act = act; q.slope = slope;
    const int vec = vec_for(C, dtype);
    if ((size_t)G * L * C / vec >= ((size_t)1 << 31)) return SSCG_ERR_UNSUPPORTED;
    q.total = (uint32_t)((size_t)G * L * C / vec);
    q.div_cg = make_fastdiv(C / vec);
    q.div_l = make_fastdiv((int)L);
    if (dtype == SSCG_BF16) launch_bwd_apply<__bf16>(q, vec, st, G);
    else launch_bwd_apply<float>(q, vec, st, G);
    SSCG_LAUNCH_CHECK();
    return SSCG_OK;
}

int sscg_finalize_bwd(const double* sums, float* coef, float* dgamma, float* dbeta, int G, int C, int chunks, long L, int overwrite, int rec_bm,
                      int rec_wm, hipStream_t st) {
    hipLaunchKernelGGL(finalize_bwd_kernel, dim3(cdiv(C, FIN_CH)), dim3(256), 0, st, sums, coef, dgamma, dbeta, G, C, chunks, L, overwrite,
                       rec_bm, rec_wm);
    SSCG_LAUNCH_CHECK();
    return SSCG_OK;
}

static bool head_ok(int C) { return C >= 16 && C <= 256 && (C & (C - 1)) == 0; }

extern "C" int sscg_norm_head_applies(int C) { return head_ok(C) ? 1 : 0; }

extern "C" int sscg_norm_head_fwd(const void* x, int dtype, const float* mean, const float* rstd, const float* gamma, const float* beta,
                                  const float* w, const float* bias, float* out, int G, int64_t L, int C, int act, float slope,
                                  void* stream) {
    if (!x || !mean || !rstd || !w || !out || G <= 0 || L <= 0 || (dtype != SSCG_F32 && dtype != SSCG_BF16)) return SSCG_ERR_BAD_ARG;
    if ((gamma != nullptr) != (beta != nullptr)) return SSCG_ERR_BAD_ARG;
    if (!head_ok(C)) return SSCG_ERR_UNSUPPORTED;
    HeadParams p = {};
    p.x = x; p.mean = mean; p.rstd = rstd; p.gamma = gamma; p.beta = beta; p.w = w; p.bias = bias; p.out = out;
    p.L = L; p.rows = (long)G * L; p.C = C; p.act = act; p.slope = slope;
    const long rows_per_block = 4L * (256 / C) * 4;
    long blocks = cdiv(p.rows, rows_per_block);
    if (blocks > 8192) blocks = 8192;
    hipStream_t st = (hipStream_t)stream;
    if (dtype == SSCG_BF16) hipLaunchKernelGGL(norm_head_fwd_kernel<__bf16>, dim3((int)blocks), dim3(256), 0, st, p);
    else hipLaunchKernelGGL(norm_head_fwd_kernel<float>, dim3((int)blocks), dim3(256), 0, st, p);
    SSCG_LAUNCH_CHECK();
    return SSCG_OK;
}

extern "C" size_t sscg_norm_head_bwd_workspace(int G, int64_t L, int C) {
    return 2 * part_bytes(G, L, C) + (size_t)G * C * 2 * sizeof(float);
}

extern "C" int sscg_norm_head_bwd(const float* dout, const float* w, const void* x, const float* mean, const float* rstd,
                                  const float* gamma, const float* beta, void* dx, float* dw, float* dbias, float* dgamma,
                                  float* dbeta, int dtype, int G, int64_t L, int C, int act, float slope, int flags, void* ws,
                                  size_t ws_bytes, void* stream) {
    if (!dout || !w || !x || !mean || !rstd || !dx || G <= 0 || L <= 0 || (dtype != SSCG_F32 && dtype != SSCG_BF16)) return SSCG_ERR_BAD_ARG;
    if (act == SSCG_ACT_TANH) return SSCG_ERR_UNSUPPORTED;
    if (!head_ok(C)) return SSCG_ERR_UNSUPPORTED;
    if (!ws || ws_bytes < sscg_norm_head_bwd_workspace(G, L, C)) return SSCG_ERR_WORKSPACE;
    hipStream_t st = (hipStream_t)stream;
    const int stats_grad = flags & 1, overwrite = (flags >> 1) & 1, overwrite_w = (flags >> 2) & 1;
    RedParams p = {};
    p.x = x; p.mean = mean; p.rstd = rstd; p.gamma = gamma; p.beta = beta;
    p.part = reinterpret_cast<double*>(ws); p.L = L; p.C = C; p.act = act; p.slope = slope;
    p.head_w = w; p.head_dout = dout;
    p.head_part = reinterpret_cast<double*>(reinterpret_cast<char*>(ws) + part_bytes(G, L, C));
    int rc = launch_reduce<RM_BWD_HEAD>(p, G, dtype, st);
    if (rc) return rc;
    RedPlan pl = plan_reduce(G, L, C, dtype);
    float* coef = reinterpret_cast<float*>(reinterpret_cast<char*>(ws) + 2 * part_bytes(G, L, C));
    hipLaunchKernelGGL(finalize_bwd_kernel, dim3(cdiv(C, FIN_CH)), dim3(256), 0, st, p.part, coef, dgamma, dbeta, G, C, pl.chunks,
                       (long)L, overwrite);
    SSCG_LAUNCH_CHECK();
    if (dw || dbias) {
        hipLaunchKernelGGL(finalize_head_kernel, dim3(cdiv(C, FIN_CH)), dim3(256), 0, st, p.head_part, dw, dbias, C, G * pl.chunks,
                           overwrite_w ? 0.f : 1.f);
        SSCG_LAUNCH_CHECK();
    }
    BwdApplyParams q = {};
    q.x = x; q.mean = mean; q.rstd = rstd; q.gamma = gamma; q.beta = beta;
    q.coef = stats_grad ? coef : nullptr;
    q.head_w = w; q.head_dout = dout;
    q.dx = dx; q.L = L; q.C = C; q.act = act; q.slope = slope;
    const int vec = vec_for(C, dtype);
    if ((size_t)G * L * C / vec >= ((size_t)1 << 31)) return SSCG_ERR_UNSUPPORTED;
    q.total = (uint32_t)((size_t)G * L * C / vec);
    q.div_cg = make_fastdiv(C / vec);
    q.div_l = make_fastdiv((int)L);
    if (dtype == SSCG_BF16) launch_bwd_apply<__bf16>(q, vec, st, G);
    else launch_bwd_apply<float>(q, vec, st, G);
    SSCG_LAUNCH_CHECK();
    return SSCG_OK;
}
```

### semi-supervised-segmentation-cyclegan_amd/csrc/sscg_internal.h

```cpp
#pragma once
#include <hip/hip_runtime.h>
#include "../../include/sscg.h"

struct sscg_bsums;
bool sscg_conv16_fwd_applies(const sscg_conv_desc* d);
bool sscg_conv16_dgrad_applies(const sscg_conv_desc* d);
bool sscg_conv16_stats_geometry(const sscg_conv_desc* d, long L, int* bm, int* wm, int* tiles_n, int* splits, int* full_tiles, int* m_tail0);
size_t sscg_conv16_fwd_workspace(const sscg_conv_desc* d, long stat_L);
size_t sscg_conv16_dgrad_workspace(const sscg_conv_desc* d);
int sscg_conv16_fwd(const sscg_conv_desc* d, const void* x, const void* w, const float* bias, void* y, double* stats, long stat_L,
                    double* xstats, void* ws, size_t ws_bytes, hipStream_t st);
int sscg_conv16_dgrad(const sscg_conv_desc* d, const void* dy, const void* wt, const float* bias, void* dx, int act, float slope,
                      void* ws, size_t ws_bytes, hipStream_t st, const sscg_bsums* bs = nullptr, const void* addend = nullptr);
bool sscg_conv16_dgrad_add_applies(const sscg_conv_desc* d);
bool sscg_conv16_bsums_geometry(const sscg_conv_desc* d, int G, long L, int* bm, int* wm, int* chunks);
bool sscg_wgrad16_applies(const sscg_conv_desc* d);
size_t sscg_wgrad16_workspace(const sscg_conv_desc* d);
int sscg_wgrad16(const sscg_conv_desc* d, const void* x, const void* dy, float* dw, float beta, void* ws, size_t ws_bytes, hipStream_t st);
bool sscg_convs_fwd_applies(const sscg_conv_desc* d);
bool sscg_convs_dgrad_applies(const sscg_conv_desc* d);
bool sscg_convs_stats_geometry(const sscg_conv_desc* d, long L, int* bm, int* wm, int* tiles_n, int* splits, int* full_tiles, int* m_tail0);
size_t sscg_convs_fwd_workspace(const sscg_conv_desc* d, long stat_L);
size_t sscg_convs_dgrad_workspace(const sscg_conv_desc* d);
int sscg_convs_fwd(const sscg_conv_desc* d, const void* x, const void* w, const float* bias, void* y, double* stats, long stat_L,
                   double* xstats, void* ws, size_t ws_bytes, hipStream_t st);
struct sscg_bn_fold_args;
bool sscg_convs_affine_applies(const sscg_conv_desc* d);
int sscg_convs_fwd_affine(const sscg_conv_desc* d, const void* x, const void* w, const float* bias, const sscg_bn_fold_args& bn, void* y,
                          void* ws, size_t ws_bytes, hipStream_t st);
bool sscg_conv16_affine_applies(const sscg_conv_desc* d);
int sscg_conv16_fwd_affine(const sscg_conv_desc* d, const void* x, const void* w, const float* bias, const sscg_bn_fold_args& bn, void* y,
                           void* ws, size_t ws_bytes, hipStream_t st);
bool sscg_convs_front_applies(const sscg_conv_desc* d, int cin);
int sscg_convs_fwd_front(const sscg_conv_desc* d, const void* xf, int cin, const float* w1, const float* b1, float slope1, void* h1,
                         const void* w, const float* bias, void* y, double* stats, long stat_L, hipStream_t st);
struct sscg_bsums {
    const void* nx;
    const void* nz;
    const float* mean;
    const float* rstd;
    const float* gamma;
    const float* beta;
    void* sums;
    int G;
    long L;
    int act;
    float slope;
};
bool sscg_convs_bsums_geometry(const sscg_conv_desc* d, int G, long L, int* bm, int* wm, int* chunks);
int sscg_convs_dgrad(const sscg_conv_desc* d, const void* dy, const void* wt, const float* bias, void* dx, int act, float slope,
                     void* ws, size_t ws_bytes, hipStream_t st, const sscg_bsums* bs = nullptr, const void* addend = nullptr);
bool sscg_bsums_records(const sscg_conv_desc* d, int G, int64_t L, int* bm, int* wm, int* chunks);
int sscg_krsc_to_crsk_split(const float* w, void* wt, int K, int RS, int C, hipStream_t st);
bool sscg_wgrads_applies(const sscg_conv_desc* d);
size_t sscg_wgrads_workspace(const sscg_conv_desc* d);
int sscg_wgrads(const sscg_conv_desc* d, const void* x, const void* dy, float* dw, float beta, void* ws, size_t ws_bytes, hipStream_t st);
bool sscg_thin1x1_fwd_applies(const sscg_conv_desc* d);
int sscg_thin1x1_fwd(const sscg_conv_desc* d, const void* x, const void* w, const float* bias, void* y, hipStream_t st);
bool sscg_thin1x1_dgrad_applies(const sscg_conv_desc* d, const float* bias, int act);
int sscg_thin1x1_dgrad(const sscg_conv_desc* d, const void* dy, const void* wt, void* dx, hipStream_t st);
int sscg_wgrad_reduce(const float* ws, float* dw, size_t n, int splits, float beta, hipStream_t st);
int sscg_finalize_bwd(const double* sums, float* coef, float* dgamma, float* dbeta, int G, int C, int chunks, long L, int overwrite, int rec_bm,
                      int rec_wm, hipStream_t st);
int sscg_finalize_conv_stats(const double* stats, int valid_tiles, int rows_per_tile, int records_per_tile, const double* xrecs,
                             int xrec, int xgroup, int G, long L, int C, float eps, float* mean, float* rstd, float* running_mean,
                             float* running_var, float momentum, hipStream_t st);
```

### semi-supervised-segmentation-cyclegan_amd/functional.py

```python
import ctypes as C

import os
import weakref

import torch

from . import _lib
from ._lib import ACT_NONE, ACT_RELU, ACT_LRELU, ACT_TANH, PAD_ZEROS, PAD_REFLECT, ConvDesc, check, lib

CL = torch.channels_last


_raw_stream = torch._C._cuda_getCurrentRawStream
_cur_dev = getattr(torch._C, "_cuda_getDevice", torch.cuda.current_device)


def _stream():
    return _raw_stream(_cur_dev())


def _ptr(t):
    return None if t is None else t.data_ptr()


# ... 596 lines not shown
FUSE_FRONT = [os.environ.get("SSCG_FUSE_FRONT", "1") != "0"]
FRONT_CALLS = [0]


def conv2d_front_applies(x, w1, w, stride, pad, dil, pad_mode):
    if not (FUSE_FRONT[0] and _MODE[0] == "f32s" and "fwd" in SPLIT_KINDS and x.dtype == torch.float32 and x.is_cuda):
        return False
    if not (tuple(w1.shape[2:]) == (1, 1) and tuple(w.shape[2:]) == (1, 1) and w1.shape[0] == w.shape[1] == 64
            and stride == 1 and pad == 0 and dil == 1 and pad_mode == PAD_ZEROS):
        return False
    n, cin, h, wd = x.shape
    key = ("front", n, cin, h, wd, w.shape[0], TUNING[0])
    v = _SPLIT_OK.get(key)
    if v is None:
        ws, plane = None, w.numel()
        d = make_desc((n, 64, h, wd), w.shape, 1, 0, 1, PAD_ZEROS, ACT_NONE, 0.0, F32, BF16X3, F32, _prec(), plane)
        v = _SPLIT_OK[key] = bool(lib.sscg_conv2d_front_applies(C.byref(d), cin))
    return v


def conv2d_front_fwd(x, w1, b1, slope1, w, bias, glc=None, want_h1=False):
    x = to_nhwc(x)
    n, cin, h, wd = x.shape
    wop, plane = weight_split(w)
    d = make_desc((n, 64, h, wd), w.shape, 1, 0, 1, PAD_ZEROS, ACT_NONE, 0.0, F32, BF16X3, F32, _prec(), plane)
    y = empty_nhwc(n, w.shape[0], h, wd, x.device, torch.float32)
    h1 = empty_nhwc(n, 64, h, wd, x.device, torch.float32) if want_h1 else None
    g = l = nb = 0
    sbuf = None
    if glc is not None:
        g, l = int(glc[0]), int(glc[1])
        nb = _stats_bytes(d, g, l)
        if not nb:
            raise _lib.SscgError("conv2d_front_fwd: no fused statistics for this geometry")
        sbuf = torch.empty(nb, dtype=torch.uint8, device=x.device)
    FRONT_CALLS[0] += 1
    w1f = w1.detach().reshape(64, cin)
    if not w1f.is_contiguous():
        w1f = w1f.contiguous()
    _timed("fwd", d, lambda: check(lib.sscg_conv2d_front_fwd(C.byref(d), x.data_ptr(), cin, w1f.data_ptr(), _ptr(b1), float(slope1), _ptr(h1),
                                                             wop.data_ptr(), _ptr(bias), y.data_ptr(), g, l, _ptr(sbuf), nb, _stream()),
                                   "sscg_conv2d_front_fwd"))
    return y, h1, ((d, sbuf) if sbuf is not None else None)


def weight_transposed(w, dtype=torch.float32):
    k, c, r, s = w.shape
    if dtype == "x3":
        wt = torch.empty(3 * w.numel(), dtype=torch.bfloat16, device=w.device)
        check(lib.sscg_weight_krsc_to_crsk(w.data_ptr(), F32, wt.data_ptr(), BF16X3, k, r * s, c, _stream()), "sscg_weight_krsc_to_crsk")
        return wt
    src = w
    if dtype == torch.bfloat16:
        src = weight_bf16(w)
    wt = torch.empty((c, k, r, s), dtype=dtype, device=w.device, memory_format=CL)
    check(lib.sscg_weight_krsc_to_crsk(src.data_ptr(), _dt(src), wt.data_ptr(), _DT[dtype], k, r * s, c, _stream()),
          "sscg_weight_krsc_to_crsk")
    return wt


def dgrad_operand(w, xshape, stride, pad, dil, dy_dtype=torch.float32):
    if dy_dtype == torch.bfloat16:
        return weight_transposed(w, torch.bfloat16)
    if _MODE[0] == "f32s" and "dgrad" in SPLIT_KINDS and split_applies(xshape, w.shape, stride, pad, dil, PAD_ZEROS, 1):
        return weight_transposed(w, "x3")
    return weight_transposed(w, torch.float32)


def _bsums_bytes(d, g, l):
    key = (id(d), "bsums", g, l)
    v = _PLAN_SIZES.get(key)
    if v is None:
        v = _PLAN_SIZES[key] = lib.sscg_conv2d_dgrad_bsums_bytes(C.byref(d), g, l)
    return v


def _dgrad_add_applies(d):
    key = (id(d), "dgrad_add")
    v = _PLAN_SIZES.get(key)
    if v is None:
        v = _PLAN_SIZES[key] = bool(lib.sscg_conv2d_dgrad_add_applies(C.byref(d)))
    return v


def conv2d_dgrad(dy, wt, xshape, wshape, stride, pad, dil, bias=None, act=ACT_NONE, slope=0.0, out_dtype=torch.float32, bsums=None,
                 addend=None, z=None):
    if act == ACT_TANH and xshape[1] > 32 and dy.dtype == torch.bfloat16 and bsums is None and addend is None:
        return act_fwd(conv2d_dgrad(dy, wt, xshape, wshape, stride, pad, dil, bias, ACT_NONE, 0.0, out_dtype), ACT_TANH, 0.0)
    wdt = BF16X3 if (wt.dim() == 1 and wt.dtype == torch.bfloat16) else _dt(wt)
    d = make_desc(xshape, wshape, stride, pad, dil, xdt=_DT[out_dtype], wdt=wdt, ydt=_dt(dy), prec=_prec("dgrad"))
    dx = empty_nhwc(d.N, d.C, d.H, d.W, dy.device, out_dtype)
    ws = _WS.get(_ws_bytes(d, "dgrad"), dy.device)
    want3 = bsums is not None or addend is not None
    plain = bias is None and act == ACT_NONE
    f32 = out_dtype == torch.float32 and dy.dtype == torch.float32
    if addend is not None and not (plain and addend.dtype == out_dtype == dy.dtype and tuple(addend.shape) == tuple(dx.shape)
                                   and addend.stride() == dx.stride() and _dgrad_add_applies(d)):
        addend = None
    joinable = addend is not None
    if joinable and not f32:
        bsums = None
    if bsums is not None:
        nx, mean, rstd, gamma, beta, (g, l, c), nact, nslope = bsums[:8]
        res = len(bsums) > 8 and bsums[8]
        nb = _bsums_bytes(d, g, l) if (plain and c == d.C and nx.dtype == out_dtype and dy.dtype == out_dtype) else 0
        if res and not (f32 and z is not None and z.dtype == torch.float32 and z.stride() == dx.stride()):
            nb = 0
        if nb:
            sums = torch.empty(nb, dtype=torch.uint8, device=dy.device)
            fused_reads = dx.numel() * dx.element_size() * (1 + (1 if res else 0) + (1 if addend is not None else 0))
            _timed("dgrad", d, lambda: check(lib.sscg_conv2d_dgrad_bsums(
                C.byref(d), dy.data_ptr(), wt.data_ptr(), dx.data_ptr(), nx.data_ptr(), z.data_ptr() if res else None, _ptr(addend),
                mean.data_ptr(), rstd.data_ptr(), _ptr(gamma), _ptr(beta), g, l, nact, nslope, sums.data_ptr(), nb, ws.data_ptr(),
                ws.numel(), _stream()), "sscg_conv2d_dgrad_bsums"), extra_bytes=fused_reads)
            return dx, (d, sums, res), joinable
    if joinable:
        _timed("dgrad", d, lambda: check(lib.sscg_conv2d_dgrad_add(C.byref(d), dy.data_ptr(), wt.data_ptr(), addend.data_ptr(), dx.data_ptr(),
                                                                   ws.data_ptr(), ws.numel(), _stream()), "sscg_conv2d_dgrad_add"),
               extra_bytes=dx.numel() * dx.element_size())
        return dx, None, True
    _timed("dgrad", d, lambda: check(lib.sscg_conv2d_dgrad(C.byref(d), dy.data_ptr(), wt.data_ptr(), _ptr(bias), dx.data_ptr(),
                                                           act, slope, ws.data_ptr(), ws.numel(), _stream()), "sscg_conv2d_dgrad"))
    return (dx, None, False) if want3 else dx


def conv2d_dgrad_param(dy, w, xshape, wshape, stride, pad, dil, bias=None, act=ACT_NONE, slope=0.0, out_dtype=torch.float32, bsums=None,
                       addend=None, z=None):
    if dy.dtype == torch.float32 and out_dtype == torch.float32 and bias is None and act == ACT_NONE:
        cp = _padded_stem(xshape, wshape, stride, pad, dil, PAD_ZEROS, 1) if (bsums is None and addend is None) else 0
        if cp:
            wp = _padded_weight(w, cp)
            xs = (xshape[0], cp, xshape[2], xshape[3])
            d0 = make_desc(xshape, wshape, stride, pad, dil, xdt=F32, wdt=BF16X3, ydt=F32, prec=_prec("dgrad"))
            return _timed("dgrad", d0, lambda: _unprofiled(lambda: resize_channels(
                conv2d_dgrad(dy, _cached_wt(wp, "x3"), xs, tuple(wp.shape), stride, pad, dil), xshape[1])))
        kp = _padded_head(xshape, wshape, stride, pad, dil)
        if kp:
            wp = _cached_copy(w, "_sscg_wpadk", lambda: _pad_filters(w.detach(), kp))
            d0 = make_desc(xshape, wshape, stride, pad, dil, xdt=F32, wdt=BF16X3, ydt=F32, prec=_prec("dgrad"))
            return _timed("dgrad", d0, lambda: _unprofiled(lambda: conv2d_dgrad(
                resize_channels(dy, kp), _cached_wt(wp, "x3"), xshape, tuple(wp.shape), stride, pad, dil, bsums=bsums, addend=addend, z=z)))
    if dy.dtype == torch.bfloat16:
        if wshape[0] % 64:
            raise _lib.SscgError("bf16 output gradients with %d channels: the bf16 conv kernels need a multiple of 64" % wshape[0])
        wt = _cached_wt(w, torch.bfloat16)
    elif (_MODE[0] == "f32s" and "dgrad" in SPLIT_KINDS and out_dtype == torch.float32
          and split_applies(xshape, wshape, stride, pad, dil, PAD_ZEROS, 1)):
        wt = _cached_wt(w, "x3")
    else:
        wt = _cached_wt(w, torch.float32)
    return conv2d_dgrad(dy, wt, xshape, wshape, stride, pad, dil, bias, act, slope, out_dtype, bsums, addend, z)


def conv2d_wgrad(x, dy, wshape, stride, pad, dil, pad_mode=PAD_ZEROS, out=None, accumulate=False):
    d = make_desc(x.shape, wshape, stride, pad, dil, pad_mode, xdt=_dt(x), ydt=_dt(dy), prec=_prec("wgrad"))
    if out is None:
        k, c, r, s = wshape
        out = torch.empty((k, c, r, s), dtype=torch.float32, device=x.device, memory_format=CL)
        accumulate = False
    ws = _WS.get(_ws_bytes(d, "wgrad"), x.device)
    _timed("wgrad", d, lambda: check(lib.sscg_conv2d_wgrad(C.byref(d), x.data_ptr(), dy.data_ptr(), out.data_ptr(),
                                                           1.0 if accumulate else 0.0, ws.data_ptr(), ws.numel(), _stream()),
                                     "sscg_conv2d_wgrad"))
    return out


def colsum(x2d_rows, cols, x, out=None, accumulate=False):
    if out is None:
        out = torch.empty(cols, dtype=torch.float32, device=x.device)
        accumulate = False
    nb = _cached_size(lib.sscg_colsum_workspace, x2d_rows, cols)
    ws = _WS.get(nb, x.device)
    check(lib.sscg_colsum(x.data_ptr(), _dt(x), out.data_ptr(), x2d_rows, cols, 1.0 if accumulate else 0.0, ws.data_ptr(),
                          ws.numel(), _stream()), "sscg_colsum")
    return out


_SIZE_CACHE = {}


def _cached_size(fn, *args):
    key = (id(fn),) + args
    v = _SIZE_CACHE.get(key)
    if v is None:
        v = _SIZE_CACHE[key] = fn(*args)
    return v


def _glc(x, per_sample):
    return _glc_shape(x.shape, per_sample)


def _glc_shape(shape, per_sample):
    n, c, h, w = shape
    if per_sample is True:
        return n, h * w, c
    k = 1 if per_sample is False else int(per_sample)
    if k < 1 or n % k:
        raise _lib.SscgError("batch of %d does not split into %d groups" % (n, k))
    return k, (n // k) * h * w, c


def norm_stats(x, per_sample, eps=1e-5, running_mean=None, running_var=None, momentum=0.1):
    g, l, c = _glc(x, per_sample)
    mean = torch.empty((g, c), dtype=torch.float32, device=x.device)
    rstd = torch.empty((g, c), dtype=torch.float32, device=x.device)
    nb = _cached_size(lib.sscg_norm_stats_workspace, g, l, c)
    ws = _WS.get(nb, x.device)
    check(lib.sscg_norm_stats(x.data_ptr(), _dt(x), g, l, c, eps, mean.data_ptr(), rstd.data_ptr(), _ptr(running_mean),
                              _ptr(running_var), momentum, ws.data_ptr(), ws.numel(), _stream()), "sscg_norm_stats")
    return mean, rstd


def norm_apply(x, mean, rstd, gamma, beta, residual, per_sample, act=ACT_NONE, slope=0.0):
    g, l, c = _glc(x, per_sample)
    y = torch.empty_like(x, memory_format=CL)
    check(lib.sscg_norm_apply(x.data_ptr(), mean.data_ptr(), rstd.data_ptr(), _ptr(gamma), _ptr(beta), _ptr(residual),
                              y.data_ptr(), _same_dtype(x, residual), g, l, c, act, slope, _stream()), "sscg_norm_apply")
    return y


def norm_bwd(dy, x, y, mean, rstd, gamma, per_sample, act, slope, stats_grad=True, want_dres=False, dgamma=None,
             dbeta=None, beta=None, overwrite=False):
    g, l, c = _glc(x, per_sample)
    dx = torch.empty_like(x, memory_format=CL)
    dres = torch.empty_like(x, memory_format=CL) if want_dres else None
    nb = _cached_size(lib.sscg_norm_bwd_workspace, g, l, c)
    ws = _WS.get(nb, x.device)
    check(lib.sscg_norm_bwd(dy.data_ptr(), x.data_ptr(), _ptr(y), mean.data_ptr(), rstd.data_ptr(), _ptr(gamma), _ptr(beta),
                            dx.data_ptr(), _ptr(dres), _ptr(dgamma), _ptr(dbeta), _same_dtype(x, dy, y), g, l, c, act, slope,
                            (1 if stats_grad else 0) | (2 if overwrite else 0), ws.data_ptr(), ws.numel(), _stream()), "sscg_norm_bwd")
    return dx, dres


def norm_bwd_from_sums(rec, dy, x, mean, rstd, gamma, beta, per_sample, act, slope, dgamma=None, dbeta=None, y=None, want_dres=False):
    d, sums = rec[0], rec[1]
    g, l, c = _glc(x, per_sample)
    dx = torch.empty_like(x, memory_format=CL)
    dres = torch.empty_like(x, memory_format=CL) if want_dres else None
    ws = _WS.get(g * c * 8, x.device)
    check(lib.sscg_norm_bwd_from_sums(C.byref(d), sums.data_ptr(), dy.data_ptr(), x.data_ptr(), _ptr(y), mean.data_ptr(), rstd.data_ptr(),
                                      _ptr(gamma), _ptr(beta), dx.data_ptr(), _ptr(dres), _ptr(dgamma), _ptr(dbeta), _same_dtype(x, dy), g, l,
                                      c, act, slope, 2, ws.data_ptr(), ws.numel(), _stream()), "sscg_norm_bwd_from_sums")
    return dx, dres


def norm_head_applies(c):
    return bool(lib.sscg_norm_head_applies(int(c)))


def norm_head_fwd(x, mean, rstd, gamma, beta, w, bias, per_sample, act, slope):
    g, l, c = _glc(x, per_sample)
    n, _, h, wd = x.shape
    out = torch.empty((n, 1, h, wd), dtype=torch.float32, device=x.device)
    check(lib.sscg_norm_head_fwd(x.data_ptr(), _dt(x), mean.data_ptr(), rstd.data_ptr(), _ptr(gamma), _ptr(beta), w.data_ptr(),
                                 _ptr(bias), out.data_ptr(), g, l, c, act, slope, _stream()), "sscg_norm_head_fwd")
    return out


def norm_head_bwd(dout, w, x, mean, rstd, gamma, beta, per_sample, act, slope, stats_grad, dwb, dgamma=None, dbeta=None):
    g, l, c = _glc(x, per_sample)
    dx = torch.empty_like(x, memory_format=CL)
    nb = _cached_size(lib.sscg_norm_head_bwd_workspace, g, l, c)
    ws = _WS.get(nb, x.device)
    check(lib.sscg_norm_head_bwd(dout.data_ptr(), w.data_ptr(), x.data_ptr(), mean.data_ptr(), rstd.data_ptr(), _ptr(gamma), _ptr(beta),
                                 dx.data_ptr(), dwb.data_ptr(), dwb.data_ptr() + 4 * c, _ptr(dgamma), _ptr(dbeta), _dt(x), g, l, c, act,
                                 slope, (1 if stats_grad else 0) | 2 | 4, ws.data_ptr(), ws.numel(), _stream()), "sscg_norm_head_bwd")
    return dx


def rstd_from_var(var, eps):
    out = torch.empty_like(var)
    check(lib.sscg_rstd_from_var(var.data_ptr(), out.data_ptr(), var.numel(), eps, _stream()), "sscg_rstd_from_var")
    return out


def act_fwd(x, act, slope=0.0):
    y = torch.empty_like(x, memory_format=torch.preserve_format)
    check(lib.sscg_act_fwd(x.data_ptr(), y.data_ptr(), _dt(x), x.numel(), act, slope, _stream()), "sscg_act_fwd")
    return y


def act_bwd(dy, y, act, slope=0.0):
    dx = torch.empty_like(y, memory_format=torch.preserve_format)
    check(lib.sscg_act_bwd(dy.data_ptr(), y.data_ptr(), dx.data_ptr(), _same_dtype(y, dy), y.numel(), act, slope, _stream()), "sscg_act_bwd")
    return dx


def add(a, b):
    y = torch.empty_like(a, memory_format=torch.preserve_format)
    check(lib.sscg_add(a.data_ptr(), b.data_ptr(), y.data_ptr(), _same_dtype(a, b), a.numel(), _stream()), "sscg_add")
    return y


def fill_(x, v):
    if x.dtype != torch.float32:
        if v != 0.0 or (x.numel() * x.element_size()) % 4:
            raise _lib.SscgError("fill_ of a %s tensor supports zero only" % x.dtype)
        check(lib.sscg_fill(x.data_ptr(), x.numel() * x.element_size() // 4, 0.0, _stream()), "sscg_fill")
        return x
    check(lib.sscg_fill(x.data_ptr(), x.numel(), float(v), _stream()), "sscg_fill")
    return x


def dropout(x, p, seed):
    y = torch.empty_like(x, memory_format=torch.preserve_format)
    check(lib.sscg_dropout(x.data_ptr(), y.data_ptr(), _dt(x), x.numel(), p, seed, _stream()), "sscg_dropout")
    return y


def gauss_noise(x, sigma, seed):
    _need_hip(x, f32_only=True)
    y = torch.empty_like(x, memory_format=torch.preserve_format)
    check(lib.sscg_gauss_noise(x.data_ptr(), y.data_ptr(), x.numel(), float(sigma), int(seed), _stream()), "sscg_gauss_noise")
    return y


def pool_out_size(h):
    o = -((-(h + 2 - 3)) // 2) + 1
    if (o - 1) * 2 >= h + 1:
        o -= 1
    return o


def maxpool_fwd(x):
    n, c, h, w = x.shape
    p, q = pool_out_size(h), pool_out_size(w)
    y = empty_nhwc(n, c, p, q, x.device, x.dtype)
    idx = torch.empty((n, c, p, q), dtype=torch.uint8, device=x.device, memory_format=CL)
    check(lib.sscg_maxpool3x3s2_fwd(x.data_ptr(), y.data_ptr(), idx.data_ptr(), _dt(x), n, h, w, c, p, q, _stream()),
          "sscg_maxpool3x3s2_fwd")
    return y, idx


def maxpool_bwd(dy, idx, xshape):
    n, c, h, w = xshape
    p, q = dy.shape[2], dy.shape[3]
    dx = empty_nhwc(n, c, h, w, dy.device, dy.dtype)
    check(lib.sscg_maxpool3x3s2_bwd(dy.data_ptr(), idx.data_ptr(), dx.data_ptr(), _dt(dy), n, h, w, c, p, q, _stream()),
          "sscg_maxpool3x3s2_bwd")
    return dx


def upsample_fwd(x, oh, ow):
    _need_hip(x, f32_only=True)
    n, c, h, w = x.shape
    y = empty_nhwc(n, c, oh, ow, x.device)
    check(lib.sscg_upsample_bilinear_fwd(x.data_ptr(), y.data_ptr(), n, h, w, c, oh, ow, _stream()), "sscg_upsample_bilinear_fwd")
    return y


def upsample_bwd(dy, h, w):
    n, c, oh, ow = dy.shape
    dx = empty_nhwc(n, c, h, w, dy.device)
    check(lib.sscg_upsample_bilinear_bwd(dy.data_ptr(), dx.data_ptr(), n, h, w, c, oh, ow, _stream()), "sscg_upsample_bilinear_bwd")
    return dx


def reflect_pad(x, pad):
    n, c, h, w = x.shape
    y = empty_nhwc(n, c, h + 2 * pad, w + 2 * pad, x.device, x.dtype)
    check(lib.sscg_reflect_pad(x.data_ptr(), y.data_ptr(), _dt(x), n, h, w, c, pad, _stream()), "sscg_reflect_pad")
    return y


def reflect_pad_bwd(dy, pad):
    n, c, oh, ow = dy.shape
    dx = empty_nhwc(n, c, oh - 2 * pad, ow - 2 * pad, dy.device, dy.dtype)
    check(lib.sscg_reflect_pad_bwd(dy.data_ptr(), dx.data_ptr(), _dt(dy), n, oh - 2 * pad, ow - 2 * pad, c, pad, _stream()),
          "sscg_reflect_pad_bwd")
    return dx


def softmax_fwd(x):
    _need_hip(x, f32_only=True)
    n, c, h, w = x.shape
    y = torch.empty_like(x, memory_format=CL)
    check(lib.sscg_softmax_fwd(x.data_ptr(), y.data_ptr(), n * h * w, c, _stream()), "sscg_softmax_fwd")
    return y


def softmax_bwd(dy, y):
    n, c, h, w = y.shape
    dx = torch.empty_like(y, memory_format=CL)
    check(lib.sscg_softmax_bwd(dy.data_ptr(), y.data_ptr(), dx.data_ptr(), n * h * w, c, _stream()), "sscg_softmax_bwd")
    return dx


def argmax_onehot(x, want_index=False):
    _need_hip(x, f32_only=True)
    x = to_nhwc(x)
    n, c, h, w = x.shape
    oh = torch.empty_like(x, memory_format=CL)
# ... 276 lines not shown


_NO_COPY_SYNC = os.environ.get("SSCG_DBG_NO_COPY_SYNC") == "1"
_IN_REFRESH = [False]


class _Copy(object):
    __slots__ = ("tag", "t", "ev", "stream", "readers", "row", "nblk")

    def __init__(self, tag, build):
        self.tag = tag
        self.stream = _stream()
        self.t = build()
        self.readers = None
        self.ev = None
        if not _IN_REFRESH[0] and not _NO_COPY_SYNC:
            self.ev = torch.cuda.Event()
            self.ev.record()
            self.readers = set()

    def get(self):
        if self.ev is not None:
            h = _stream()
            if h != self.stream and h not in self.readers:
                torch.cuda.current_stream().wait_event(self.ev)
                self.readers.add(h)
        return self.t

    def retire(self):
        if self.readers:
            dev = self.t.device
            for h in self.readers:
                self.t.record_stream(_stream_object(dev, h))


def _cached_copy(w, attr, build):
    tag = _wtag(w)
    ent = getattr(w, attr, None)
    if ent is None or ent.tag != tag:
        if ent is not None:
            ent.retire()
        ent = _Copy(tag, build)
        try:
            setattr(w, attr, ent)
        except AttributeError:
            pass
    return ent.get()


def _cached_wt(w, dtype=torch.float32):
    kind = "tx3" if dtype == "x3" else ("t16" if dtype == torch.bfloat16 else "t32")
    _note_user(w, kind)
    attr = {"tx3": "_sscg_wtx3", "t16": "_sscg_wt16", "t32": "_sscg_wt"}[kind]
    return _cached_copy(w, attr, lambda: weight_transposed(w, dtype))


def weight_bf16(w):
    _note_user(w, "w16")
    opt = getattr(w, "_sscg_opt", None)
    opt = opt() if opt is not None else None
    if opt is not None:
        return opt.shadow_view(w)
    return _cached_copy(w, "_sscg_w16", lambda: cast(w, torch.bfloat16))


def _split3_copy(w):
    n = w.numel()
    t = torch.empty(3 * n, dtype=torch.bfloat16, device=w.device)
    src = w if w.is_contiguous(memory_format=CL) else w.contiguous(memory_format=CL)
    check(lib.sscg_split3(src.data_ptr(), t.data_ptr(), n, n, _stream()), "sscg_split3")
    return t


def weight_split(w):
    _note_user(w, "wx3")
    opt = getattr(w, "_sscg_opt", None)
    opt = opt() if opt is not None else None
    if opt is not None and hasattr(opt, "split_view"):
        return opt.split_view(w)
    return _cached_copy(w, "_sscg_wx3", lambda: _split3_copy(w)), w.numel()


def _acc_target(param):
    acc = getattr(param, "_sscg_grad", None)
    if acc is not None:
        param._sscg_touched = True
    return acc


def _running_stats(running_mean, running_var, per_sample):
    if running_mean is not None and per_sample is not True:
        return running_mean, running_var
    return None, None


def _conv_stats_fwd(x, w, bias, geom, out_f32, norm, fallback=True):
    stride, pad, dil, pad_mode = geom
    per_sample, eps, rmean, rvar, momentum = norm
    n, _, h, wd = x.shape
    p, q = conv_out_size(h, w.shape[2], stride, pad, dil), conv_out_size(wd, w.shape[3], stride, pad, dil)
    glc = _glc_shape((n, w.shape[0], p, q), per_sample)
    y, mean, rstd = conv2d_fwd_norm(x, w, bias, stride, pad, dil, pad_mode, out_f32, glc, eps, rmean, rvar, momentum)
    if mean is None and fallback:
        mean, rstd = norm_stats(y, per_sample, eps, *_running_stats(rmean, rvar, per_sample), momentum)
    return y, mean, rstd, glc


def _add_into(acc, src_ptr, count):
    check(lib.sscg_add(acc.data_ptr(), src_ptr, acc.data_ptr(), F32, count, _stream()), "sscg_add")


def _arena_add(device, acc, src_ptr, count, ref, keep):
    run_on_side_stream(device, (keep,), lambda: _add_into(acc, src_ptr, count), lane=getattr(ref, "_sscg_lane", 0), defer=True)


class Conv2dFn(torch.autograd.Function):

    @staticmethod
    def forward(ctx, x, w, bias, stride, pad, dil, pad_mode, act, slope, out_f32, norm, grad):
        x = to_nhwc(x)
        mean = rstd = None
        if norm is not None and act == ACT_NONE:
            y, mean, rstd, _ = _conv_stats_fwd(x, w, bias, (stride, pad, dil, pad_mode), out_f32, norm, fallback=False)
        else:
            y = conv2d_fwd(x, w, bias, stride, pad, dil, pad_mode, act, slope, out_f32)
        ctx.cfg = (stride, pad, dil, pad_mode, act, slope)
        ctx.has_bias = bias is not None
        ctx.wref = w
        ctx.bref = bias
        ctx.counted = _note_use(w, bias) if grad and ctx.needs_input_grad[1] else ()
        ctx.save_for_backward(x, w, y if act != ACT_NONE else None)
        ctx.set_materialize_grads(False)
        if norm is None:
            return y
        if mean is None:
            return y, None, None
        ctx.mark_non_differentiable(mean, rstd)
        return y, mean, rstd

    @staticmethod
    def backward(ctx, dy, *_unused):
        if dy is None:
            return (None,) * 12
        x, w, y = ctx.saved_tensors
        stride, pad, dil, pad_mode, act, slope = ctx.cfg
        dy = to_nhwc(dy)
        if act != ACT_NONE:
            dy = act_bwd(dy, y, act, slope)
        dx, dw, db = _conv_backward(dy, x, w, ctx.wref, ctx.bref if ctx.has_bias else None, (stride, pad, dil, pad_mode),
                                    ctx.needs_input_grad[0], ctx.needs_input_grad[1], ctx.has_bias and ctx.needs_input_grad[2], ctx.counted)
        return dx, dw, db, None, None, None, None, None, None, None, None, None


def _conv_backward(dy, x, w, wref, bref, geom, want_x, want_w, want_b, counted):
    stride, pad, dil, pad_mode = geom
    dx = None
    if want_x:
        if pad_mode == PAD_REFLECT:
            raise _lib.SscgError("input gradient through a reflection-padded conv: use ReflectPadFn + pad=0 conv")
        fuse = FUSE_BSUMS[0] and stride == 1 and x.dtype == dy.dtype and (x.dtype == torch.float32 or FUSE_BSUMS_BF16[0])
        join = getattr(x, "_sscg_join", None) if FUSE_JOIN[0] else None
        addend = None
        if join is not None:
            addend = join[0].take(join[1])
            info = join[0].norm if (fuse and addend is not None) else None
        else:
            info = getattr(x, "_sscg_norm", None) if fuse else None
        if info is not None and len(info) > 8 and info[8] and x.dtype != torch.float32:
            info = None
        if info is not None or addend is not None:
            dx, rec, joined = conv2d_dgrad_param(dy, wref, x.shape, w.shape, stride, pad, dil, out_dtype=x.dtype, bsums=info, addend=addend, z=x)
            if addend is not None and not joined:
                rec = None
            if rec is not None:
                dx._sscg_bsums = (rec, dx._version)
            if join is not None:
                if joined:
                    join[0].folded = (join[1], dx)
                else:
                    join[0].deposit(join[1], dx)
        else:
            dx = conv2d_dgrad_param(dy, wref, x.shape, w.shape, stride, pad, dil, out_dtype=x.dtype)
            if join is not None:
                join[0].deposit(join[1], dx)
    dw, db = _param_grads(x, dy, dy, w.shape, geom, wref, bref, want_w, want_b)
    _note_done(counted)
    return dx, dw, db


def _param_grads(a, b, dy, wshape, geom, wref, bref, want_w, want_b):
    stride, pad, dil, pad_mode = geom
    dw = db = None
    wacc = _acc_target(wref) if want_w else None
    bacc = _acc_target(bref) if want_b else None
    n, k, p, q = dy.shape

    def arena_grads():
        if wacc is not None:
            conv2d_wgrad(a, b, wshape, stride, pad, dil, pad_mode, out=wacc, accumulate=True)
        if bacc is not None:
            colsum(n * p * q, k, dy, out=bacc, accumulate=True)

    if wacc is not None or bacc is not None:
        run_on_side_stream(dy.device, (a, b), arena_grads, lane=getattr(wref, "_sscg_lane", 0), defer=True)
    if want_w and wacc is None:
        dw = conv2d_wgrad(a, b, wshape, stride, pad, dil, pad_mode)
    if want_b and bacc is None:
        db = colsum(n * p * q, k, dy)
    return dw, db


class ConvTranspose2dFn(torch.autograd.Function):

    @staticmethod
    def forward(ctx, x, w, bias, stride, pad, out_pad, act, slope, out_f32=False):
        x = to_nhwc(x)
        n, cin, h, wd = x.shape
        cin2, cout, r, s = w.shape
        oh = (h - 1) * stride - 2 * pad + (r - 1) + out_pad + 1
        ow = (wd - 1) * stride - 2 * pad + (s - 1) + out_pad + 1
        if conv_out_size(oh, r, stride, pad, 1) != h or conv_out_size(ow, s, stride, pad, 1) != wd:
            raise _lib.SscgError("unsupported ConvTranspose2d geometry")
        y = conv2d_dgrad_param(x, w, (n, cout, oh, ow), (cin, cout, r, s), stride, pad, 1, bias, act, slope,
                               out_dtype=_out_dtype(out_f32))
        ctx.cfg = (stride, pad, act, slope)
        ctx.has_bias = bias is not None
        ctx.wref, ctx.bref = w, bias
        ctx.save_for_backward(x, w, y if act != ACT_NONE else None)
        return y

    @staticmethod
    def backward(ctx, dy):
        x, w, y = ctx.saved_tensors
        stride, pad, act, slope = ctx.cfg
        dy = to_nhwc(dy)
        if act != ACT_NONE:
            dy = act_bwd(dy, y, act, slope)
        dx = None
        if ctx.needs_input_grad[0]:
            dx = conv2d_fwd(dy, w, None, stride, pad, 1, out_f32=(x.dtype == torch.float32))
        dw, db = _param_grads(dy, x, dy, w.shape, (stride, pad, 1, PAD_ZEROS), ctx.wref, ctx.bref,
                              ctx.needs_input_grad[1], ctx.has_bias and ctx.needs_input_grad[2])
        return dx, dw, db, None, None, None, None, None, None


class NormActFn(torch.autograd.Function):

    @staticmethod
    def forward(ctx, x, gamma, beta, residual, running_mean, running_var, per_sample, training, momentum, eps, act, slope,
                pre_mean=None, pre_rstd=None):
        x = to_nhwc(x)
        if residual is not None:
            residual = to_nhwc(residual)
        use_batch_stats = training or running_mean is None
        if use_batch_stats and pre_mean is not None:
            mean, rstd = pre_mean, pre_rstd
        elif use_batch_stats:
            rmean, rvar = _running_stats(running_mean, running_var, per_sample) if training else (None, None)
            mean, rstd = norm_stats(x, per_sample, eps, rmean, rvar, momentum)
        else:
            per_sample = False
            mean = running_mean.view(1, -1)
            rstd = rstd_from_var(running_var, eps).view(1, -1)
        y = norm_apply(x, mean, rstd, gamma, beta, residual, per_sample, act, slope)
        ctx.cfg = (per_sample, act, slope, use_batch_stats, residual is not None)
        ctx.gref, ctx.betaref = gamma, beta
        need_y = act != ACT_NONE and (residual is not None or act not in (ACT_RELU, ACT_LRELU))
        ctx.save_for_backward(x, y if need_y else None, mean, rstd, gamma, beta)
        return y

    @staticmethod
    def backward(ctx, dy):
        x, y, mean, rstd, gamma, beta = ctx.saved_tensors
        per_sample, act, slope, stats_grad, has_res = ctx.cfg
        dx, ret_g, ret_b, dres = _norm_backward(to_nhwc(dy), x, y, mean, rstd, gamma, beta, ctx.gref, ctx.betaref, per_sample, act, slope,
                                                stats_grad, gamma is not None and ctx.needs_input_grad[1],
                                                has_res and ctx.needs_input_grad[3])
        if not ctx.needs_input_grad[0]:
            dx = None
        return dx, ret_g, ret_b, dres, None, None, None, None, None, None, None, None, None, None


def _norm_backward(dy, x, y, mean, rstd, gamma, beta, gref, betaref, per_sample, act, slope, stats_grad, want_g, want_dres):
    dgamma = dbeta = dgb = None
    ret_g = ret_b = None
    gacc = bacc = None
    rec = getattr(dy, "_sscg_bsums", None)
    from_sums = (rec is not None and rec[1] == dy._version and stats_grad and act in (ACT_NONE, ACT_RELU, ACT_LRELU)
                 and (y is not None) == bool(rec[0][2]))
    if want_g:
        gacc = _acc_target(gref)
        bacc = _acc_target(betaref)
        fin = rec[0][3] if (from_sums and len(rec[0]) > 3) else None
        if fin is not None:
            dgb = fin[fin.numel() - 2 * gamma.numel():].view(2, gamma.numel())
        else:
            dgb = torch.empty((2, gamma.numel()), dtype=torch.float32, device=gamma.device)
        dgamma, dbeta = dgb[0], dgb[1]
        if gacc is None or bacc is None:
            gacc = bacc = None
            ret_g, ret_b = dgamma, dbeta
    if from_sums:
        dx, dres = norm_bwd_from_sums(rec[0], dy, x, mean, rstd, gamma, beta, per_sample, act, slope, dgamma, dbeta, y=y, want_dres=want_dres)
    else:
        dx, dres = norm_bwd(dy, x, y, mean, rstd, gamma, per_sample, act, slope, stats_grad,
                            want_dres=want_dres, dgamma=dgamma, dbeta=dbeta, beta=beta, overwrite=True)
    if gacc is not None:
        n_c = gacc.numel()
        if bacc.data_ptr() == gacc.data_ptr() + 4 * n_c:
            _arena_add(dy.device, gacc, dgb.data_ptr(), 2 * n_c, gref, dgb)
        else:
            def both():
                _add_into(gacc, dgamma.data_ptr(), n_c)
                _add_into(bacc, dbeta.data_ptr(), n_c)
            run_on_side_stream(dy.device, (dgb,), both, lane=getattr(gref, "_sscg_lane", 0), defer=True)
    return dx, ret_g, ret_b, dres


class ConvNormActFn(torch.autograd.Function):

    @staticmethod
    def forward(ctx, x, w, bias, gamma, beta, residual, running_mean, running_var, cfg):
        stride, pad, dil, pad_mode, per_sample, eps, momentum, act, slope, grad = cfg
        x = to_nhwc(x)
        if residual is not None:
            residual = to_nhwc(residual)
        y, mean, rstd, glc = _conv_stats_fwd(x, w, bias, (stride, pad, dil, pad_mode), False,
                                             (per_sample, eps, running_mean, running_var, momentum))
        z = norm_apply(y, mean, rstd, gamma, beta, residual, per_sample, act, slope)
        ctx.cfg = cfg
        ctx.has_bias = bias is not None
        ctx.has_res = residual is not None
        ctx.wref, ctx.bref, ctx.gref, ctx.betaref = w, bias, gamma, beta
        ctx.counted = _note_use(w, bias) if grad and ctx.needs_input_grad[1] else ()
        need_z = act != ACT_NONE and (residual is not None or act not in (ACT_RELU, ACT_LRELU))
        ctx.save_for_backward(x, w, y, z if need_z else None, mean, rstd, gamma, beta)
        ctx.res_join = getattr(residual, "_sscg_join", None) if (residual is not None and FUSE_JOIN[0]) else None
        if (FUSE_BSUMS[0] and grad and any(ctx.needs_input_grad) and act in (ACT_NONE, ACT_RELU, ACT_LRELU)
                and (residual is None or FUSE_JOIN[0])):
            z._sscg_norm = (y, mean, rstd, gamma, beta, glc, act, slope, need_z)
        return z

    @staticmethod
    def backward(ctx, dz):
        x, w, y, z, mean, rstd, gamma, beta = ctx.saved_tensors
        stride, pad, dil, pad_mode, per_sample, eps, momentum, act, slope, _ = ctx.cfg
        ni = ctx.needs_input_grad
        dy, ret_g, ret_b, dres = _norm_backward(to_nhwc(dz), y, z, mean, rstd, gamma, beta, ctx.gref, ctx.betaref, per_sample, act, slope,
                                                True, gamma is not None and ni[3], ctx.has_res and ni[5])
        if ctx.res_join is not None and dres is not None:
            ctx.res_join[0].deposit(ctx.res_join[1], dres)
        dx, dw, db = _conv_backward(dy, x, w, ctx.wref, ctx.bref if ctx.has_bias else None, (stride, pad, dil, pad_mode),
                                    ni[0], ni[1], ctx.has_bias and ni[2], ctx.counted)
        return dx, dw, db, ret_g, ret_b, dres, None, None, None


def _head_fwd(y, mean, rstd, gamma, beta, hw, hbias, per_sample, act, slope):
    hw32 = hw.detach().reshape(-1)
    if hw32.dtype != torch.float32:
        hw32 = hw32.float()
    return norm_head_fwd(y, mean, rstd, gamma, beta, hw32, hbias, per_sample, act, slope), hw32


def _head_backward(dout, y, mean, rstd, gamma, beta, hw32, gref, betaref, hwref, hbref, per_sample, act, slope, want_g, want_hw, want_hb):
    dout = dout.contiguous()
    if dout.dtype != torch.float32:
        dout = dout.float()
    c = hw32.numel()
    dgb = torch.empty((2, c), dtype=torch.float32, device=y.device) if want_g else None
    dwb = torch.empty(c + 1, dtype=torch.float32, device=y.device)
    dy = norm_head_bwd(dout, hw32, y, mean, rstd, gamma, beta, per_sample, act, slope, True, dwb,
                       dgb[0] if want_g else None, dgb[1] if want_g else None)
    ret_hw = ret_hb = ret_g = ret_b = None
    hwacc = _acc_target(hwref) if want_hw else None
    hbacc = _acc_target(hbref) if want_hb else None
    if want_hw and hwacc is None:
        ret_hw = dwb[:c].reshape(hwref.shape).to(hwref.dtype)
    if want_hb and hbacc is None:
        ret_hb = dwb[c:c + 1].clone()
    gacc = _acc_target(gref) if want_g else None
    bacc = _acc_target(betaref) if want_g else None
    if want_g and (gacc is None or bacc is None):
        gacc = bacc = None
        ret_g, ret_b = dgb[0], dgb[1]
    if hwacc is not None:
        _arena_add(y.device, hwacc, dwb.data_ptr(), c, hwref, dwb)
    if hbacc is not None:
        _arena_add(y.device, hbacc, dwb.data_ptr() + 4 * c, 1, hbref, dwb)
    if gacc is not None:
        _arena_add(y.device, gacc, dgb.data_ptr(), c, gref, dgb)
        _arena_add(y.device, bacc, dgb.data_ptr() + 4 * c, c, betaref, dgb)
    return dy, ret_g, ret_b, ret_hw, ret_hb


class ConvNormActHeadFn(torch.autograd.Function):

    @staticmethod
    def forward(ctx, x, w, bias, gamma, beta, hw, hbias, running_mean, running_var, cfg):
        stride, pad, dil, pad_mode, per_sample, eps, momentum, act, slope, grad = cfg
        x = to_nhwc(x)
        y, mean, rstd, _ = _conv_stats_fwd(x, w, bias, (stride, pad, dil, pad_mode), False,
                                           (per_sample, eps, running_mean, running_var, momentum))
        out, hw32 = _head_fwd(y, mean, rstd, gamma, beta, hw, hbias, per_sample, act, slope)
        ctx.cfg = cfg
        ctx.has_bias = bias is not None
        ctx.has_hbias = hbias is not None
        ctx.wref, ctx.bref, ctx.gref, ctx.betaref, ctx.hwref, ctx.hbref = w, bias, gamma, beta, hw, hbias
        ctx.counted = _note_use(w, bias) if grad and ctx.needs_input_grad[1] else ()
        ctx.save_for_backward(x, w, y, mean, rstd, gamma, beta, hw32)
        return out

    @staticmethod
    def backward(ctx, dout):
        x, w, y, mean, rstd, gamma, beta, hw32 = ctx.saved_tensors
        stride, pad, dil, pad_mode, per_sample, eps, momentum, act, slope, _ = ctx.cfg
        ni = ctx.needs_input_grad
        dy, ret_g, ret_b, ret_hw, ret_hb = _head_backward(dout, y, mean, rstd, gamma, beta, hw32, ctx.gref, ctx.betaref, ctx.hwref, ctx.hbref,
                                                          per_sample, act, slope, gamma is not None and ni[3], ni[5], ctx.has_hbias and ni[6])
        dx, dw, db = _conv_backward(dy, x, w, ctx.wref, ctx.bref if ctx.has_bias else None, (stride, pad, dil, pad_mode),
                                    ni[0], ni[1], ctx.has_bias and ni[2], ctx.counted)
        return dx, dw, db, ret_g, ret_b, ret_hw, ret_hb, None, None, None


class PixelDiscFn(torch.autograd.Function):

    @staticmethod
    def forward(ctx, x, w1, b1, w, bias, gamma, beta, hw, hbias, running_mean, running_var, cfg):
        slope1, per_sample, eps, momentum, act, slope, grad = cfg
        x = to_nhwc(x)
        n, _, h, wd = x.shape
        g, l, c = _glc_shape((n, w.shape[0], h, wd), per_sample)
        will = grad and any(ctx.needs_input_grad)
        y, h1, cs = conv2d_front_fwd(x, w1, b1, slope1, w, bias, (g, l, c), want_h1=will)
        mean, rstd = norm_stats_from_conv(cs, (g, l, c), eps, *_running_stats(running_mean, running_var, per_sample), momentum)
        out, hw32 = _head_fwd(y, mean, rstd, gamma, beta, hw, hbias, per_sample, act, slope)
        ctx.cfg = cfg
        ctx.has_b1, ctx.has_bias, ctx.has_hbias = b1 is not None, bias is not None, hbias is not None
        ctx.w1ref, ctx.b1ref, ctx.wref, ctx.bref, ctx.gref, ctx.betaref, ctx.hwref, ctx.hbref = w1, b1, w, bias, gamma, beta, hw, hbias
        ctx.counted1 = _note_use(w1, b1) if grad and ctx.needs_input_grad[1] else ()
        ctx.counted = _note_use(w, bias) if grad and ctx.needs_input_grad[3] else ()
        if will:
            ctx.save_for_backward(x, w1, h1, w, y, mean, rstd, gamma, beta, hw32)
        return out

    @staticmethod
    def backward(ctx, dout):
        x, w1, h1, w, y, mean, rstd, gamma, beta, hw32 = ctx.saved_tensors
        slope1, per_sample, eps, momentum, act, slope, _ = ctx.cfg
        ni = ctx.needs_input_grad
        dy, ret_g, ret_b, ret_hw, ret_hb = _head_backward(dout, y, mean, rstd, gamma, beta, hw32, ctx.gref, ctx.betaref, ctx.hwref, ctx.hbref,
                                                          per_sample, act, slope, gamma is not None and ni[5], ni[7], ctx.has_hbias and ni[8])
        geom = (1, 0, 1, PAD_ZEROS)
        front = ni[0] or ni[1] or (ctx.has_b1 and ni[2])
        dh1, dw, db = _conv_backward(dy, h1, w, ctx.wref, ctx.bref if ctx.has_bias else None, geom, front, ni[3], ctx.has_bias and ni[4],
                                     ctx.counted)
        dx = dw1 = db1 = None
        if front:
            dh1 = act_bwd(dh1, h1, ACT_LRELU, slope1)
            dx, dw1, db1 = _conv_backward(dh1, x, w1, ctx.w1ref, ctx.b1ref if ctx.has_b1 else None, geom, ni[0], ni[1], ctx.has_b1 and ni[2],
                                          ctx.counted1)
        return dx, dw1, db1, dw, db, ret_g, ret_b, ret_hw, ret_hb, None, None, None


def pixel_disc(x, w1, b1, slope1, w, bias, gamma, beta, hw, hbias, running_mean, running_var, per_sample, eps, momentum, act, slope):
    return PixelDiscFn.apply(x, w1, b1, w, bias, gamma, beta, hw, hbias, running_mean, running_var,
                             (slope1, per_sample, eps, momentum, act, slope, torch.is_grad_enabled()))


def conv_norm_act_head(x, w, bias, stride, pad, dil, pad_mode, gamma, beta, hw, hbias, running_mean, running_var, per_sample, eps,
                       momentum, act, slope):
    return ConvNormActHeadFn.apply(x, w, bias, gamma, beta, hw, hbias, running_mean, running_var,
                                   (stride, pad, dil, pad_mode, per_sample, eps, momentum, act, slope, torch.is_grad_enabled()))


class ActFn(torch.autograd.Function):
    @staticmethod
    def forward(ctx, x, act, slope):
        _need_hip(x)
        if not (x.is_contiguous() or x.is_contiguous(memory_format=CL)):
            x = x.contiguous()
        y = act_fwd(x, act, slope)
        ctx.cfg = (act, slope)
        ctx.save_for_backward(y)
        return y

    @staticmethod
    def backward(ctx, dy):
        (y,) = ctx.saved_tensors
        act, slope = ctx.cfg
        if dy.stride() != y.stride():
            dy = to_nhwc(dy) if y.is_contiguous(memory_format=CL) else dy.contiguous()
        return act_bwd(dy, y, act, slope), None, None


class AddFn(torch.autograd.Function):
    @staticmethod
    def forward(ctx, a, b):
        a, b = to_nhwc(a), to_nhwc(b)
        return add(a, b)

    @staticmethod
    def backward(ctx, dy):
        return dy, dy


FUSE_JOIN = [os.environ.get("SSCG_FUSE_JOIN", "1") != "0"]
# ... 494 lines not shown
```

Measured before the change: 67.60 img/s.

## Emit split-bf16 gradient planes from norm backward for reuse in weight gradient

The norm backward apply kernel now also writes the three-piece bf16 split of the fp32 input gradient directly into a planes buffer. The split-bf16 weight-gradient path then consumes these planes instead of running its own split3 pass over dy. This removes one full read of dy and one extra kernel launch per conv-norm layer. In exchange the norm kernel writes an extra 6 bytes per element, and a separate planes tensor is allocated and has to stay alive until the side-stream wgrad has run.

Result: no change. 67.63 img/s, median of 2 (+0.0%).

```diff
diff --git a/include/sscg.h b/include/sscg.h
--- a/include/sscg.h
+++ b/include/sscg.h
@@ -73,6 +73,10 @@
 int sscg_conv2d_wgrad(const sscg_conv_desc* d, const void* x, const void* dy, float* dw, float beta, void* ws,
                       size_t ws_bytes, void* stream);
 
+int sscg_conv2d_wgrad_takes_dy_planes(const sscg_conv_desc* d);
+int sscg_conv2d_wgrad_planes(const sscg_conv_desc* d, const void* x, const void* dy, const void* dy_planes, float* dw, float beta,
+                             void* ws, size_t ws_bytes, void* stream);
+
 int sscg_weight_krsc_to_crsk(const void* w, int w_dtype, void* wt, int wt_dtype, int K, int RS, int C, void* stream);
 typedef struct sscg_wt_job {
     const void* w;
@@ -104,12 +108,20 @@
 int sscg_norm_bwd_from_sums(const sscg_conv_desc* d, const void* sums, const void* dy, const void* x, const void* y, const float* mean,
                             const float* rstd, const float* gamma, const float* beta, void* dx, void* dres, float* dgamma, float* dbeta,
                             int dtype, int G, int64_t L, int C, int act, float slope, int flags, void* ws, size_t ws_bytes, void* stream);
+int sscg_norm_bwd_planes_applies(int dtype, int G, int64_t L, int C);
+int sscg_norm_bwd_from_sums_planes(const sscg_conv_desc* d, const void* sums, const void* dy, const void* x, const void* y,
+                                   const float* mean, const float* rstd, const float* gamma, const float* beta, void* dx, void* dres,
+                                   float* dgamma, float* dbeta, int dtype, int G, int64_t L, int C, int act, float slope, int flags,
+                                   void* ws, size_t ws_bytes, void* dx_planes, void* stream);
 
 int sscg_rstd_from_var(const float* var, float* rstd, int n, float eps, void* stream);
 size_t sscg_norm_bwd_workspace(int G, int64_t L, int C);
 int sscg_norm_bwd(const void* dy, const void* x, const void* y, const float* mean, const float* rstd,
                   const float* gamma, const float* beta, void* dx, void* dres, float* dgamma, float* dbeta, int dtype, int G,
                   int64_t L, int C, int act, float slope, int stats_grad, void* ws, size_t ws_bytes, void* stream);
+int sscg_norm_bwd_planes(const void* dy, const void* x, const void* y, const float* mean, const float* rstd,
+                         const float* gamma, const float* beta, void* dx, void* dres, float* dgamma, float* dbeta, int dtype, int G,
+                         int64_t L, int C, int act, float slope, int stats_grad, void* ws, size_t ws_bytes, void* dx_planes, void* stream);
 
 int sscg_norm_head_applies(int C);
 int sscg_norm_head_fwd(const void* x, int dtype, const float* mean, const float* rstd, const float* gamma, const float* beta,
diff --git a/semi-supervised-segmentation-cyclegan_amd/_lib.py b/semi-supervised-segmentation-cyclegan_amd/_lib.py
--- a/semi-supervised-segmentation-cyclegan_amd/_lib.py
+++ b/semi-supervised-segmentation-cyclegan_amd/_lib.py
@@ -53,8 +53,12 @@
     "sscg_conv2d_dgrad_add_applies": (_i, [_dp]),
     "sscg_conv2d_dgrad_add": (_i, [_dp, _p, _p, _p, _p, _p, _sz, _p]),
     "sscg_norm_bwd_from_sums": (_i, [_dp, _p, _p, _p, _p, _p, _p, _p, _p, _p, _p, _p, _p, _i, _i, _i64, _i, _i, _f, _i, _p, _sz, _p]),
+    "sscg_norm_bwd_planes_applies": (_i, [_i, _i, _i64, _i]),
+    "sscg_norm_bwd_from_sums_planes": (_i, [_dp, _p, _p, _p, _p, _p, _p, _p, _p, _p, _p, _p, _p, _i, _i, _i64, _i, _i, _f, _i, _p, _sz, _p, _p]),
     "sscg_conv2d_wgrad_workspace": (_sz, [_dp]),
     "sscg_conv2d_wgrad": (_i, [_dp, _p, _p, _p, _f, _p, _sz, _p]),
+    "sscg_conv2d_wgrad_takes_dy_planes": (_i, [_dp]),
+    "sscg_conv2d_wgrad_planes": (_i, [_dp, _p, _p, _p, _p, _f, _p, _sz, _p]),
     "sscg_weight_krsc_to_crsk": (_i, [_p, _i, _p, _i, _i, _i, _i, _p]),
     "sscg_weight_krsc_to_crsk_batch": (_i, [_p, _i, _i, _p]),
     "sscg_split3": (_i, [_p, _p, _i64, _i64, _p]),
@@ -68,6 +72,7 @@
     "sscg_rstd_from_var": (_i, [_p, _p, _i, _f, _p]),
     "sscg_norm_bwd_workspace": (_sz, [_i, _i64, _i]),
     "sscg_norm_bwd": (_i, [_p, _p, _p, _p, _p, _p, _p, _p, _p, _p, _p, _i, _i, _i64, _i, _i, _f, _i, _p, _sz, _p]),
+    "sscg_norm_bwd_planes": (_i, [_p, _p, _p, _p, _p, _p, _p, _p, _p, _p, _p, _i, _i, _i64, _i, _i, _f, _i, _p, _sz, _p, _p]),
     "sscg_norm_head_applies": (_i, [_i]),
     "sscg_norm_head_fwd": (_i, [_p, _i, _p, _p, _p, _p, _p, _p, _p, _i, _i64, _i, _i, _f, _p]),
     "sscg_norm_head_bwd_workspace": (_sz, [_i, _i64, _i]),
diff --git a/semi-supervised-segmentation-cyclegan_amd/csrc/common.h b/semi-supervised-segmentation-cyclegan_amd/csrc/common.h
--- a/semi-supervised-segmentation-cyclegan_amd/csrc/common.h
+++ b/semi-supervised-segmentation-cyclegan_amd/csrc/common.h
@@ -47,6 +47,20 @@
     h = __builtin_bit_cast(bf16x8, ph);
     m = __builtin_bit_cast(bf16x8, pm);
     l = __builtin_bit_cast(bf16x8, pl);
+}
+
+typedef uint32_t sscg_u32x2 __attribute__((ext_vector_type(2)));
+__device__ __forceinline__ void sscg_split4(const float (&x)[4], sscg_u32x2& h, sscg_u32x2& m, sscg_u32x2& l) {
+#pragma unroll
+    for (int w = 0; w < 2; ++w) {
+        float a = x[2 * w], b = x[2 * w + 1];
+        asm volatile("" : "+v"(a), "+v"(b));
+        const uint32_t hh = sscg_cvt_pk_bf16(a, b);
+        const float ra = a - __builtin_bit_cast(float, hh << 16), rb = b - __builtin_bit_cast(float, hh & 0xffff0000u);
+        const uint32_t mm = sscg_cvt_pk_bf16(ra, rb);
+        const float sa = ra - __builtin_bit_cast(float, mm << 16), sb = rb - __builtin_bit_cast(float, mm & 0xffff0000u);
+        h[w] = hh; m[w] = mm; l[w] = sscg_cvt_pk_bf16(sa, sb);
+    }
 }
 
 template <typename T> __device__ __forceinline__ float ld1(const T* p);
diff --git a/semi-supervised-segmentation-cyclegan_amd/csrc/conv_split.hip b/semi-supervised-segmentation-cyclegan_amd/csrc/conv_split.hip
--- a/semi-supervised-segmentation-cyclegan_amd/csrc/conv_split.hip
+++ b/semi-supervised-segmentation-cyclegan_amd/csrc/conv_split.hip
@@ -1930,16 +1930,20 @@
     return ((wgs_planes_bytes(d) + 255) & ~(size_t)255) + part;
 }
 
-int sscg_wgrads(const sscg_conv_desc* d, const void* x, const void* dy, float* dw, float beta, void* ws, size_t ws_bytes, hipStream_t st) {
-    if (wgf_applies(d)) return launch_wgf(d, x, dy, dw, beta, ws, ws_bytes, st);
+bool sscg_wgrads_reads_planes(const sscg_conv_desc* d) { return sscg_wgrads_applies(d) && !wgf_applies(d); }
+
+int sscg_wgrads(const sscg_conv_desc* d, const void* x, const void* dy, float* dw, float beta, void* ws, size_t ws_bytes, hipStream_t st,
+                const void* dy3) {
+    if (wgf_applies(d)) return dy3 ? SSCG_ERR_UNSUPPORTED : launch_wgf(d, x, dy, dw, beta, ws, ws_bytes, st);
     if (!ws || ws_bytes < sscg_wgrads_workspace(d)) return SSCG_ERR_WORKSPACE;
     const WgsPlan pl = plan_wgs(d);
     const size_t nx = (size_t)d->N * d->H * d->W * d->C, ny = (size_t)d->N * d->P * d->Q * d->K;
     bf16* x3 = reinterpret_cast<bf16*>(ws);
-    bf16* y3 = x3 + 3 * nx;
+    const bf16* y3 = dy3 ? reinterpret_cast<const bf16*>(dy3) : x3 + 3 * nx;
     float* part = reinterpret_cast<float*>(reinterpret_cast<char*>(ws) + ((wgs_planes_bytes(d) + 255) & ~(size_t)255));
     hipLaunchKernelGGL(split3_kernel, dim3(cdiv((long)((nx + 7) / 8), 256)), dim3(256), 0, st, reinterpret_cast<const float*>(x), x3, nx, nx);
-    hipLaunchKernelGGL(split3_kernel, dim3(cdiv((long)((ny + 7) / 8), 256)), dim3(256), 0, st, reinterpret_cast<const float*>(dy), y3, ny, ny);
+    if (!dy3)
+        hipLaunchKernelGGL(split3_kernel, dim3(cdiv((long)((ny + 7) / 8), 256)), dim3(256), 0, st, reinterpret_cast<const float*>(dy), x3 + 3 * nx, ny, ny);
     SSCG_LAUNCH_CHECK();
     WgsParams p = {};
     p.x3 = x3; p.dy3 = y3; p.xplane = (long)nx; p.yplane = (long)ny;
diff --git a/semi-supervised-segmentation-cyclegan_amd/csrc/conv_wgrad.hip b/semi-supervised-segmentation-cyclegan_amd/csrc/conv_wgrad.hip
--- a/semi-supervised-segmentation-cyclegan_amd/csrc/conv_wgrad.hip
+++ b/semi-supervised-segmentation-cyclegan_amd/csrc/conv_wgrad.hip
@@ -635,6 +635,23 @@
     return (size_t)pl.splits * d->K * d->R * d->S * d->C * sizeof(float);
 }
 
+static bool wgrad_reads_planes(const sscg_conv_desc* d) {
+    if (d->N <= 0 || d->C <= 0 || d->K <= 0 || !wg_dt_ok(d->x_dtype) || !wg_dt_ok(d->y_dtype)) return false;
+    if ((long)d->N * d->H * d->W * (long)d->C >= (1L << 31) || (long)d->N * d->P * d->Q * (long)d->K >= (1L << 31)) return false;
+    if (thin_wgrad_applies(d) && thin_wgrad_supported_T(d->K < d->C ? d->K : d->C)) return false;
+    if (sscg_wgrad16_applies(d)) return false;
+    return sscg_wgrads_reads_planes(d);
+}
+
+extern "C" int sscg_conv2d_wgrad_takes_dy_planes(const sscg_conv_desc* d) { return (d && wgrad_reads_planes(d)) ? 1 : 0; }
+
+extern "C" int sscg_conv2d_wgrad_planes(const sscg_conv_desc* d, const void* x, const void* dy, const void* dy_planes, float* dw, float beta,
+                                        void* ws, size_t ws_bytes, void* stream) {
+    if (!d || !x || !dy || !dy_planes || !dw) return SSCG_ERR_BAD_ARG;
+    if (!wgrad_reads_planes(d)) return SSCG_ERR_UNSUPPORTED;
+    return sscg_wgrads(d, x, dy, dw, beta, ws, ws_bytes, (hipStream_t)stream, dy_planes);
+}
+
 extern "C" int sscg_conv2d_wgrad(const sscg_conv_desc* d, const void* x, const void* dy, float* dw, float beta,
                                  void* ws, size_t ws_bytes, void* stream) {
     if (!d || !x || !dy || !dw) return SSCG_ERR_BAD_ARG;
diff --git a/semi-supervised-segmentation-cyclegan_amd/csrc/norm.hip b/semi-supervised-segmentation-cyclegan_amd/csrc/norm.hip
--- a/semi-supervised-segmentation-cyclegan_amd/csrc/norm.hip
+++ b/semi-supervised-segmentation-cyclegan_amd/csrc/norm.hip
@@ -528,8 +528,10 @@
     }
 }
 
-template <typename T, int VEC, int U>
-__global__ __launch_bounds__(256) void norm_bwd_apply_slab_kernel(BwdApplyParams p, int cw_shift, int rows_per_chunk) {
+template <typename T, int VEC, int U, bool PL = false>
+__global__ __launch_bounds__(256) void norm_bwd_apply_slab_kernel(BwdApplyParams p, int cw_shift, int rows_per_chunk, __bf16* __restrict__ dx3,
+                                                                  long plane) {
+    static_assert(!PL || (VEC == 4 && sizeof(T) == 4), "planes: fp32 tensors, four-channel groups");
     const int tid = threadIdx.x;
     const int col = tid & ((1 << cw_shift) - 1), rl = tid >> cw_shift, rw = 256 >> cw_shift;
     const int c = (((int)blockIdx.y << cw_shift) + col) * VEC;
@@ -598,6 +600,14 @@
                 }
                 stv<T, VEC>(pdx + o, gx);
                 if (pdres) stv<T, VEC>(pdres + o, gr);
+                if constexpr (PL) {
+                    sscg_u32x2 h, m, l;
+                    sscg_split4(gx, h, m, l);
+                    __bf16* q = dx3 + base + o;
+                    *reinterpret_cast<sscg_u32x2*>(q) = h;
+                    *reinterpret_cast<sscg_u32x2*>(q + plane) = m;
+                    *reinterpret_cast<sscg_u32x2*>(q + 2 * plane) = l;
+                }
             }
         }
     }
@@ -868,17 +878,33 @@
     return part_bytes(G, L, C) + (size_t)G * C * 2 * sizeof(float);
 }
 
+static bool bwd_planes_ok(int dtype, int G, long L, int C) {
+    return dtype == SSCG_F32 && vec_for(C, dtype) == 4 && plan_slab(G, L, C, 4, 4).ok;
+}
+
+extern "C" int sscg_norm_bwd_planes_applies(int dtype, int G, int64_t L, int C) {
+    return (G > 0 && L > 0 && C > 0 && bwd_planes_ok(dtype, G, (long)L, C)) ? 1 : 0;
+}
+
 template <typename T>
-static void launch_bwd_apply(const BwdApplyParams& q, int vec, hipStream_t st, int G = 0) {
+static void launch_bwd_apply(const BwdApplyParams& q, int vec, hipStream_t st, int G = 0, void* dx3 = nullptr) {
     static const int u8 = getenv("SSCG_NORM_SLAB_U8B") ? atoi(getenv("SSCG_NORM_SLAB_U8B")) : 1;
     const int U = vec == 8 ? u8 : 4;
     const SlabPlan sp = (G > 0 && U > 0) ? plan_slab(G, q.L, q.C, vec, U) : SlabPlan{false, 0, 1, 1, 0};
     if (sp.ok) {
         const dim3 grid(sp.chunks, sp.slabs, G);
-        if (vec == 8 && U == 1) hipLaunchKernelGGL((norm_bwd_apply_slab_kernel<T, 8, 1>), grid, dim3(256), 0, st, q, sp.cw_shift, sp.rows_per_chunk);
-        else if (vec == 8 && U == 2) hipLaunchKernelGGL((norm_bwd_apply_slab_kernel<T, 8, 2>), grid, dim3(256), 0, st, q, sp.cw_shift, sp.rows_per_chunk);
+        __bf16* const no3 = nullptr;
+        if constexpr (sizeof(T) == 4) {
+            if (dx3) {
+                hipLaunchKernelGGL((norm_bwd_apply_slab_kernel<T, 4, 4, true>), grid, dim3(256), 0, st, q, sp.cw_shift, sp.rows_per_chunk,
+                                   reinterpret_cast<__bf16*>(dx3), (long)G * q.L * q.C);
+                return;
+            }
+        }
+        if (vec == 8 && U == 1) hipLaunchKernelGGL((norm_bwd_apply_slab_kernel<T, 8, 1>), grid, dim3(256), 0, st, q, sp.cw_shift, sp.rows_per_chunk, no3, 0L);
+        else if (vec == 8 && U == 2) hipLaunchKernelGGL((norm_bwd_apply_slab_kernel<T, 8, 2>), grid, dim3(256), 0, st, q, sp.cw_shift, sp.rows_per_chunk, no3, 0L);
         else if (vec == 8) return launch_bwd_apply<T>(q, vec, st);
-        else hipLaunchKernelGGL((norm_bwd_apply_slab_kernel<T, 4, 4>), grid, dim3(256), 0, st, q, sp.cw_shift, sp.rows_per_chunk);
+        else hipLaunchKernelGGL((norm_bwd_apply_slab_kernel<T, 4, 4>), grid, dim3(256), 0, st, q, sp.cw_shift, sp.rows_per_chunk, no3, 0L);
         return;
     }
     if (vec == 8) hipLaunchKernelGGL((norm_bwd_apply_kernel<T, 8>), dim3(ew_grid(q.total)), dim3(256), 0, st, q);
@@ -886,9 +912,9 @@
     else hipLaunchKernelGGL((norm_bwd_apply_kernel<T, 1>), dim3(ew_grid(q.total)), dim3(256), 0, st, q);
 }
 
-extern "C" int sscg_norm_bwd(const void* dy, const void* x, const void* y, const float* mean, const float* rstd,
-                             const float* gamma, const float* beta, void* dx, void* dres, float* dgamma, float* dbeta, int dtype, int G,
-                             int64_t L, int C, int act, float slope, int stats_grad, void* ws, size_t ws_bytes, void* stream) {
+static int norm_bwd_impl(const void* dy, const void* x, const void* y, const float* mean, const float* rstd,
+                         const float* gamma, const float* beta, void* dx, void* dres, float* dgamma, float* dbeta, int dtype, int G,
+                         int64_t L, int C, int act, float slope, int stats_grad, void* ws, size_t ws_bytes, void* stream, void* dx3) {
     if (!dy || !x || !mean || !rstd || !dx || G <= 0 || L <= 0 || C <= 0 || (dtype != SSCG_F32 && dtype != SSCG_BF16)) return SSCG_ERR_BAD_ARG;
     if (act == SSCG_ACT_TANH && !y) return SSCG_ERR_BAD_ARG;
     if (act != SSCG_ACT_NONE && !y && dres) return SSCG_ERR_BAD_ARG;
@@ -920,15 +946,32 @@
     q.div_cg = make_fastdiv(C / vec);
     q.div_l = make_fastdiv((int)L);
     if (dtype == SSCG_BF16) launch_bwd_apply<__bf16>(q, vec, st, G);
-    else launch_bwd_apply<float>(q, vec, st, G);
+    else launch_bwd_apply<float>(q, vec, st, G, dx3);
     SSCG_LAUNCH_CHECK();
     return SSCG_OK;
 }
 
-extern "C" int sscg_norm_bwd_from_sums(const sscg_conv_desc* d, const void* sums, const void* dy, const void* x, const void* y,
-                                       const float* mean, const float* rstd, const float* gamma, const float* beta, void* dx, void* dres,
-                                       float* dgamma, float* dbeta, int dtype, int G, int64_t L, int C, int act, float slope, int flags,
-                                       void* ws, size_t ws_bytes, void* stream) {
+extern "C" int sscg_norm_bwd(const void* dy, const void* x, const void* y, const float* mean, const float* rstd,
+                             const float* gamma, const float* beta, void* dx, void* dres, float* dgamma, float* dbeta, int dtype, int G,
+                             int64_t L, int C, int act, float slope, int stats_grad, void* ws, size_t ws_bytes, void* stream) {
+    return norm_bwd_impl(dy, x, y, mean, rstd, gamma, beta, dx, dres, dgamma, dbeta, dtype, G, L, C, act, slope, stats_grad, ws, ws_bytes,
+                         stream, nullptr);
+}
+
+extern "C" int sscg_norm_bwd_planes(const void* dy, const void* x, const void* y, const float* mean, const float* rstd,
+                                    const float* gamma, const float* beta, void* dx, void* dres, float* dgamma, float* dbeta, int dtype,
+                                    int G, int64_t L, int C, int act, float slope, int stats_grad, void* ws, size_t ws_bytes,
+                                    void* dx_planes, void* stream) {
+    if (!dx_planes) return SSCG_ERR_BAD_ARG;
+    if (G <= 0 || L <= 0 || C <= 0 || !bwd_planes_ok(dtype, G, (long)L, C)) return SSCG_ERR_UNSUPPORTED;
+    return norm_bwd_impl(dy, x, y, mean, rstd, gamma, beta, dx, dres, dgamma, dbeta, dtype, G, L, C, act, slope, stats_grad, ws, ws_bytes,
+                         stream, dx_planes);
+}
+
+static int norm_bwd_from_sums_impl(const sscg_conv_desc* d, const void* sums, const void* dy, const void* x, const void* y,
+                                   const float* mean, const float* rstd, const float* gamma, const float* beta, void* dx, void* dres,
+                                   float* dgamma, float* dbeta, int dtype, int G, int64_t L, int C, int act, float slope, int flags,
+                                   void* ws, size_t ws_bytes, void* stream, void* dx3) {
     if (!d || !sums || !dy || !x || !mean || !rstd || !dx || G <= 0 || L <= 0 || C <= 0 || (dtype != SSCG_F32 && dtype != SSCG_BF16)) return SSCG_ERR_BAD_ARG;
     if (act != SSCG_ACT_NONE && act != SSCG_ACT_RELU && act != SSCG_ACT_LRELU) return SSCG_ERR_UNSUPPORTED;
     if (act != SSCG_ACT_NONE && !y && dres) return SSCG_ERR_BAD_ARG;
@@ -950,9 +993,27 @@
     q.div_cg = make_fastdiv(C / vec);
     q.div_l = make_fastdiv((int)L);
     if (dtype == SSCG_BF16) launch_bwd_apply<__bf16>(q, vec, st, G);
-    else launch_bwd_apply<float>(q, vec, st, G);
+    else launch_bwd_apply<float>(q, vec, st, G, dx3);
     SSCG_LAUNCH_CHECK();
     return SSCG_OK;
+}
+
+extern "C" int sscg_norm_bwd_from_sums(const sscg_conv_desc* d, const void* sums, const void* dy, const void* x, const void* y,
+                                       const float* mean, const float* rstd, const float* gamma, const float* beta, void* dx, void* dres,
+                                       float* dgamma, float* dbeta, int dtype, int G, int64_t L, int C, int act, float slope, int flags,
+                                       void* ws, size_t ws_bytes, void* stream) {
+    return norm_bwd_from_sums_impl(d, sums, dy, x, y, mean, rstd, gamma, beta, dx, dres, dgamma, dbeta, dtype, G, L, C, act, slope, flags, ws,
+                                   ws_bytes, stream, nullptr);
+}
+
+extern "C" int sscg_norm_bwd_from_sums_planes(const sscg_conv_desc* d, const void* sums, const void* dy, const void* x, const void* y,
+                                              const float* mean, const float* rstd, const float* gamma, const float* beta, void* dx,
+                                              void* dres, float* dgamma, float* dbeta, int dtype, int G, int64_t L, int C, int act,
+                                              float slope, int flags, void* ws, size_t ws_bytes, void* dx_planes, void* stream) {
+    if (!dx_planes) return SSCG_ERR_BAD_ARG;
+    if (G <= 0 || L <= 0 || C <= 0 || !bwd_planes_ok(dtype, G, (long)L, C)) return SSCG_ERR_UNSUPPORTED;
+    return norm_bwd_from_sums_impl(d, sums, dy, x, y, mean, rstd, gamma, beta, dx, dres, dgamma, dbeta, dtype, G, L, C, act, slope, flags, ws,
+                                   ws_bytes, stream, dx_planes);
 }
 
 int sscg_finalize_bwd(const double* sums, float* coef, float* dgamma, float* dbeta, int G, int C, int chunks, long L, int overwrite, int rec_bm,
diff --git a/semi-supervised-segmentation-cyclegan_amd/csrc/sscg_internal.h b/semi-supervised-segmentation-cyclegan_amd/csrc/sscg_internal.h
--- a/semi-supervised-segmentation-cyclegan_amd/csrc/sscg_internal.h
+++ b/semi-supervised-segmentation-cyclegan_amd/csrc/sscg_internal.h
@@ -54,7 +54,9 @@
 int sscg_krsc_to_crsk_split(const float* w, void* wt, int K, int RS, int C, hipStream_t st);
 bool sscg_wgrads_applies(const sscg_conv_desc* d);
 size_t sscg_wgrads_workspace(const sscg_conv_desc* d);
-int sscg_wgrads(const sscg_conv_desc* d, const void* x, const void* dy, float* dw, float beta, void* ws, size_t ws_bytes, hipStream_t st);
+bool sscg_wgrads_reads_planes(const sscg_conv_desc* d);
+int sscg_wgrads(const sscg_conv_desc* d, const void* x, const void* dy, float* dw, float beta, void* ws, size_t ws_bytes, hipStream_t st,
+                const void* dy3 = nullptr);
 bool sscg_thin1x1_fwd_applies(const sscg_conv_desc* d);
 int sscg_thin1x1_fwd(const sscg_conv_desc* d, const void* x, const void* w, const float* bias, void* y, hipStream_t st);
 bool sscg_thin1x1_dgrad_applies(const sscg_conv_desc* d, const float* bias, int act);
diff --git a/semi-supervised-segmentation-cyclegan_amd/functional.py b/semi-supervised-segmentation-cyclegan_amd/functional.py
--- a/semi-supervised-segmentation-cyclegan_amd/functional.py
+++ b/semi-supervised-segmentation-cyclegan_amd/functional.py
@@ -772,13 +772,42 @@
     return conv2d_dgrad(dy, wt, xshape, wshape, stride, pad, dil, bias, act, slope, out_dtype, bsums, addend, z)
 
 
-def conv2d_wgrad(x, dy, wshape, stride, pad, dil, pad_mode=PAD_ZEROS, out=None, accumulate=False):
+FUSE_DY_PLANES = [os.environ.get("SSCG_FUSE_DY_PLANES", "0") == "1"]
+
+
+def _takes_dy_planes(d):
+    key = (id(d), "dy_planes")
+    v = _PLAN_SIZES.get(key)
+    if v is None:
+        v = _PLAN_SIZES[key] = bool(lib.sscg_conv2d_wgrad_takes_dy_planes(C.byref(d)))
+    return v
+
+
+def dy_planes_apply(xshape, wshape, stride, pad, dil, pad_mode, glc):
+    if not FUSE_DY_PLANES[0] or _prec("wgrad") != 2:
+        return False
+    d = make_desc(xshape, wshape, stride, pad, dil, pad_mode, xdt=F32, ydt=F32, prec=2)
+    if not _takes_dy_planes(d):
+        return False
+    key = ("norm_planes",) + tuple(glc)
+    v = _PLAN_SIZES.get(key)
+    if v is None:
+        v = _PLAN_SIZES[key] = bool(lib.sscg_norm_bwd_planes_applies(F32, *glc))
+    return v
+
+
+def conv2d_wgrad(x, dy, wshape, stride, pad, dil, pad_mode=PAD_ZEROS, out=None, accumulate=False, dy_planes=None):
     d = make_desc(x.shape, wshape, stride, pad, dil, pad_mode, xdt=_dt(x), ydt=_dt(dy), prec=_prec("wgrad"))
     if out is None:
         k, c, r, s = wshape
         out = torch.empty((k, c, r, s), dtype=torch.float32, device=x.device, memory_format=CL)
         accumulate = False
     ws = _WS.get(_ws_bytes(d, "wgrad"), x.device)
+    if dy_planes is not None and _takes_dy_planes(d):
+        _timed("wgrad", d, lambda: check(lib.sscg_conv2d_wgrad_planes(C.byref(d), x.data_ptr(), dy.data_ptr(), dy_planes.data_ptr(),
+                                                                      out.data_ptr(), 1.0 if accumulate else 0.0, ws.data_ptr(),
+                                                                      ws.numel(), _stream()), "sscg_conv2d_wgrad_planes"))
+        return out
     _timed("wgrad", d, lambda: check(lib.sscg_conv2d_wgrad(C.byref(d), x.data_ptr(), dy.data_ptr(), out.data_ptr(),
                                                            1.0 if accumulate else 0.0, ws.data_ptr(), ws.numel(), _stream()),
                                      "sscg_conv2d_wgrad"))
@@ -841,24 +870,37 @@
 
 
 def norm_bwd(dy, x, y, mean, rstd, gamma, per_sample, act, slope, stats_grad=True, want_dres=False, dgamma=None,
-             dbeta=None, beta=None, overwrite=False):
+             dbeta=None, beta=None, overwrite=False, planes=None):
     g, l, c = _glc(x, per_sample)
     dx = torch.empty_like(x, memory_format=CL)
     dres = torch.empty_like(x, memory_format=CL) if want_dres else None
     nb = _cached_size(lib.sscg_norm_bwd_workspace, g, l, c)
     ws = _WS.get(nb, x.device)
+    if planes is not None:
+        check(lib.sscg_norm_bwd_planes(dy.data_ptr(), x.data_ptr(), _ptr(y), mean.data_ptr(), rstd.data_ptr(), _ptr(gamma), _ptr(beta),
+                                       dx.data_ptr(), _ptr(dres), _ptr(dgamma), _ptr(dbeta), _same_dtype(x, dy, y), g, l, c, act, slope,
+                                       (1 if stats_grad else 0) | (2 if overwrite else 0), ws.data_ptr(), ws.numel(), planes.data_ptr(),
+                                       _stream()), "sscg_norm_bwd_planes")
+        return dx, dres
     check(lib.sscg_norm_bwd(dy.data_ptr(), x.data_ptr(), _ptr(y), mean.data_ptr(), rstd.data_ptr(), _ptr(gamma), _ptr(beta),
                             dx.data_ptr(), _ptr(dres), _ptr(dgamma), _ptr(dbeta), _same_dtype(x, dy, y), g, l, c, act, slope,
                             (1 if stats_grad else 0) | (2 if overwrite else 0), ws.data_ptr(), ws.numel(), _stream()), "sscg_norm_bwd")
     return dx, dres
 
 
-def norm_bwd_from_sums(rec, dy, x, mean, rstd, gamma, beta, per_sample, act, slope, dgamma=None, dbeta=None, y=None, want_dres=False):
+def norm_bwd_from_sums(rec, dy, x, mean, rstd, gamma, beta, per_sample, act, slope, dgamma=None, dbeta=None, y=None, want_dres=False,
+                       planes=None):
     d, sums = rec[0], rec[1]
     g, l, c = _glc(x, per_sample)
     dx = torch.empty_like(x, memory_format=CL)
     dres = torch.empty_like(x, memory_format=CL) if want_dres else None
     ws = _WS.get(g * c * 8, x.device)
+    if planes is not None:
+        check(lib.sscg_norm_bwd_from_sums_planes(C.byref(d), sums.data_ptr(), dy.data_ptr(), x.data_ptr(), _ptr(y), mean.data_ptr(),
+                                                 rstd.data_ptr(), _ptr(gamma), _ptr(beta), dx.data_ptr(), _ptr(dres), _ptr(dgamma),
+                                                 _ptr(dbeta), _same_dtype(x, dy), g, l, c, act, slope, 2, ws.data_ptr(), ws.numel(),
+                                                 planes.data_ptr(), _stream()), "sscg_norm_bwd_from_sums_planes")
+        return dx, dres
     check(lib.sscg_norm_bwd_from_sums(C.byref(d), sums.data_ptr(), dy.data_ptr(), x.data_ptr(), _ptr(y), mean.data_ptr(), rstd.data_ptr(),
                                       _ptr(gamma), _ptr(beta), dx.data_ptr(), _ptr(dres), _ptr(dgamma), _ptr(dbeta), _same_dtype(x, dy), g, l,
                                       c, act, slope, 2, ws.data_ptr(), ws.numel(), _stream()), "sscg_norm_bwd_from_sums")
@@ -1441,7 +1483,7 @@
         return dx, dw, db, None, None, None, None, None, None, None, None, None
 
 
-def _conv_backward(dy, x, w, wref, bref, geom, want_x, want_w, want_b, counted):
+def _conv_backward(dy, x, w, wref, bref, geom, want_x, want_w, want_b, counted, dy_planes=None):
     stride, pad, dil, pad_mode = geom
     dx = None
     if want_x:
@@ -1472,12 +1514,12 @@
             dx = conv2d_dgrad_param(dy, wref, x.shape, w.shape, stride, pad, dil, out_dtype=x.dtype)
             if join is not None:
                 join[0].deposit(join[1], dx)
-    dw, db = _param_grads(x, dy, dy, w.shape, geom, wref, bref, want_w, want_b)
+    dw, db = _param_grads(x, dy, dy, w.shape, geom, wref, bref, want_w, want_b, dy_planes)
     _note_done(counted)
     return dx, dw, db
 
 
-def _param_grads(a, b, dy, wshape, geom, wref, bref, want_w, want_b):
+def _param_grads(a, b, dy, wshape, geom, wref, bref, want_w, want_b, b_planes=None):
     stride, pad, dil, pad_mode = geom
     dw = db = None
     wacc = _acc_target(wref) if want_w else None
@@ -1486,14 +1528,14 @@
 
     def arena_grads():
         if wacc is not None:
-            conv2d_wgrad(a, b, wshape, stride, pad, dil, pad_mode, out=wacc, accumulate=True)
+            conv2d_wgrad(a, b, wshape, stride, pad, dil, pad_mode, out=wacc, accumulate=True, dy_planes=b_planes)
         if bacc is not None:
             colsum(n * p * q, k, dy, out=bacc, accumulate=True)
 
     if wacc is not None or bacc is not None:
-        run_on_side_stream(dy.device, (a, b), arena_grads, lane=getattr(wref, "_sscg_lane", 0), defer=True)
+        run_on_side_stream(dy.device, (a, b, b_planes), arena_grads, lane=getattr(wref, "_sscg_lane", 0), defer=True)
     if want_w and wacc is None:
-        dw = conv2d_wgrad(a, b, wshape, stride, pad, dil, pad_mode)
+        dw = conv2d_wgrad(a, b, wshape, stride, pad, dil, pad_mode, dy_planes=b_planes)
     if want_b and bacc is None:
         db = colsum(n * p * q, k, dy)
     return dw, db
@@ -1570,7 +1612,7 @@
         return dx, ret_g, ret_b, dres, None, None, None, None, None, None, None, None, None, None
 
 
-def _norm_backward(dy, x, y, mean, rstd, gamma, beta, gref, betaref, per_sample, act, slope, stats_grad, want_g, want_dres):
+def _norm_backward(dy, x, y, mean, rstd, gamma, beta, gref, betaref, per_sample, act, slope, stats_grad, want_g, want_dres, planes=None):
     dgamma = dbeta = dgb = None
     ret_g = ret_b = None
     gacc = bacc = None
@@ -1590,10 +1632,11 @@
             gacc = bacc = None
             ret_g, ret_b = dgamma, dbeta
     if from_sums:
-        dx, dres = norm_bwd_from_sums(rec[0], dy, x, mean, rstd, gamma, beta, per_sample, act, slope, dgamma, dbeta, y=y, want_dres=want_dres)
+        dx, dres = norm_bwd_from_sums(rec[0], dy, x, mean, rstd, gamma, beta, per_sample, act, slope, dgamma, dbeta, y=y, want_dres=want_dres,
+                                      planes=planes)
     else:
         dx, dres = norm_bwd(dy, x, y, mean, rstd, gamma, per_sample, act, slope, stats_grad,
-                            want_dres=want_dres, dgamma=dgamma, dbeta=dbeta, beta=beta, overwrite=True)
+                            want_dres=want_dres, dgamma=dgamma, dbeta=dbeta, beta=beta, overwrite=True, planes=planes)
     if gacc is not None:
         n_c = gacc.numel()
         if bacc.data_ptr() == gacc.data_ptr() + 4 * n_c:
@@ -1635,12 +1678,17 @@
         x, w, y, z, mean, rstd, gamma, beta = ctx.saved_tensors
         stride, pad, dil, pad_mode, per_sample, eps, momentum, act, slope, _ = ctx.cfg
         ni = ctx.needs_input_grad
-        dy, ret_g, ret_b, dres = _norm_backward(to_nhwc(dz), y, z, mean, rstd, gamma, beta, ctx.gref, ctx.betaref, per_sample, act, slope,
-                                                True, gamma is not None and ni[3], ctx.has_res and ni[5])
+        dz = to_nhwc(dz)
+        planes = None
+        if (ni[1] and x.dtype == torch.float32 and y.dtype == torch.float32 and dz.dtype == torch.float32
+                and dy_planes_apply(x.shape, w.shape, stride, pad, dil, pad_mode, _glc(y, per_sample))):
+            planes = torch.empty(3 * y.numel(), dtype=torch.bfloat16, device=y.device)
+        dy, ret_g, ret_b, dres = _norm_backward(dz, y, z, mean, rstd, gamma, beta, ctx.gref, ctx.betaref, per_sample, act, slope,
+                                                True, gamma is not None and ni[3], ctx.has_res and ni[5], planes=planes)
         if ctx.res_join is not None and dres is not None:
             ctx.res_join[0].deposit(ctx.res_join[1], dres)
         dx, dw, db = _conv_backward(dy, x, w, ctx.wref, ctx.bref if ctx.has_bias else None, (stride, pad, dil, pad_mode),
-                                    ni[0], ni[1], ctx.has_bias and ni[2], ctx.counted)
+                                    ni[0], ni[1], ctx.has_bias and ni[2], ctx.counted, dy_planes=planes)
         return dx, dw, db, ret_g, ret_b, dres, None, None, None
 
 
```
